# axruff/cuda-flow3d

Hardware: AMD Instinct MI355X
Metric: Mvoxels/s full pyramid solve (higher is better)
Workload: dtype f32; 1 GPU; 512^3 synthetic translated-Gaussian float32 pair (BASELINE config 4), full coarse-to-fine pyramid (40 levels x 40 outer x 5 inner, alpha 7.5, median 5^3, Gaussian sigma 2), frames resident in HBM (value = device-resident rate); parallelism=1 GPU

## Files before the change

### cuda-flow3d_amd/__init__.py

```python
import atexit
import collections
import contextlib
import ctypes as C
import os
import weakref

import numpy as np

_HERE = os.path.dirname(os.path.abspath(__file__))
_LIBDIR = os.environ.get("F3D_LIBDIR") or os.path.join(_HERE, "lib")

DEFAULT_PARAMS = dict(
    warp_levels_count=40, warp_scale_factor=0.95, outer_iterations_count=40, inner_iterations_count=5,
    equation_alpha=7.5, equation_smoothness=0.001, equation_data=0.001, median_radius=5, gaussian_sigma=2.0,
)


class F3dError(RuntimeError):
    pass


class Size4(C.Structure):
    _fields_ = [("width", C.c_size_t), ("height", C.c_size_t), ("depth", C.c_size_t), ("pitch", C.c_size_t)]

# ... 291 lines not shown
        "f3d_flow_create": [C.POINTER(C.c_void_p)], "f3d_flow_initialize": [C.c_void_p, _sz, _sz, _sz],
        "f3d_flow_compute": [C.c_void_p, _fp, _fp, pp, C.c_int, _fp, _fp, _fp],
        "f3d_flow_upload": [C.c_void_p, _fp, _fp],
        "f3d_flow_compute_resident": [C.c_void_p, pp, C.c_int, _fp],
        "f3d_flow_download": [C.c_void_p, _fp, _fp, _fp],
        "f3d_flow_container": [C.c_void_p, C.POINTER(Size4)], "f3d_flow_destroy": [C.c_void_p],
        "f3d_flow_set_level_stats": [C.c_void_p, C.c_int], "f3d_flow_level_stat_count": [C.c_void_p, C.POINTER(_sz)],
        "f3d_flow_level_stat": [C.c_void_p, _sz, C.POINTER(LevelStat)],
        "f3d_flow_final_residual": [C.c_void_p, C.POINTER(C.c_double), C.POINTER(C.c_double)],
        "f3d_flow_trajectory_begin": [C.c_void_p], "f3d_flow_trajectory_append": [C.c_void_p],
        "f3d_flow_trajectory_download": [C.c_void_p, _fp, _fp, _fp, C.POINTER(C.c_ulonglong)],
        "f3d_flow_trajectory_end": [C.c_void_p],
        "f3d_flow_strain_compute": [C.c_void_p, C.c_int, C.c_uint, C.POINTER(_fp), C.POINTER(StrainStats)],
        "f3d_flow_strain_end": [C.c_void_p],
        "f3d_flow_window_strain_compute": [C.c_void_p, C.c_int, C.c_uint, C.c_uint, C.c_uint, C.POINTER(_fp),
                                           C.POINTER(WindowStrainStats)],
        "f3d_flow_window_strain_end": [C.c_void_p],
        "f3d_flow_principal_compute": [C.c_void_p, C.c_int, C.c_uint, C.POINTER(_fp), C.POINTER(PrincipalStats)],
        "f3d_flow_principal_end": [C.c_void_p],
        "f3d_flow_polar_compute": [C.c_void_p, C.c_int, C.c_uint, C.POINTER(_fp), C.POINTER(PolarStats)],
        "f3d_flow_polar_end": [C.c_void_p],
        "f3d_flow_window_principal_compute": [C.c_void_p, C.c_int, C.c_uint, C.c_uint, C.c_uint, C.POINTER(_fp),
                                              C.POINTER(PrincipalStats)],
        "f3d_flow_window_principal_end": [C.c_void_p],
        "f3d_flow_window_polar_compute": [C.c_void_p, C.c_int, C.c_uint, C.c_uint, C.c_uint, C.POINTER(_fp), C.POINTER(PolarStats)],
        "f3d_flow_window_polar_end": [C.c_void_p],
        "f3d_flow_inverse_compute": [C.c_void_p, C.c_int, C.c_uint, C.c_float, C.POINTER(_fp), C.POINTER(InverseStats)],
        "f3d_flow_inverse_end": [C.c_void_p],
        "f3d_flow_match_compute": [C.c_void_p, C.c_int, C.c_uint, C.c_uint, C.c_float, C.POINTER(_fp), C.POINTER(CorrelationStats)],
        "f3d_flow_match_end": [C.c_void_p],
        "f3d_motion_solve": [C.POINTER(MotionSums), C.c_int, C.POINTER(MotionFit)],
        "f3d_motion_solve_labels": [C.POINTER(MotionSums), _sz, C.c_int, C.c_ulonglong, C.POINTER(C.c_double), C.POINTER(MotionFit),
                                    C.POINTER(C.c_int)],
        "f3d_flow_motion_compute": [C.c_void_p, C.c_int, C.c_int, C.c_float, C.POINTER(_fp), C.POINTER(MotionFit),
                                    C.POINTER(MotionResidual)],
        "f3d_flow_motion_end": [C.c_void_p],
        "f3d_flow_label_motion_compute": [C.c_void_p, C.c_int, C.POINTER(C.c_int), _sz, C.c_int, C.c_ulonglong, C.POINTER(_fp),
                                          C.POINTER(MotionFit), C.POINTER(C.c_int), C.POINTER(C.c_double), C.POINTER(LabelInfo)],
        "f3d_flow_label_motion_end": [C.c_void_p],
        "f3d_contact_kinematics": [C.POINTER(Contact), _sz, C.POINTER(_sz), C.POINTER(MotionFit), C.POINTER(C.c_int), _sz, C.c_ulonglong,
                                   C.POINTER(ContactKinematics)],
        "f3d_flow_contacts_compute": [C.c_void_p, C.c_int, C.POINTER(C.c_int), _sz, C.POINTER(C.POINTER(Contact)), C.POINTER(_sz),
                                      C.POINTER(ContactInfo)],
        "f3d_flow_contacts_end": [C.c_void_p],
        "f3d_flow_labels_compute": [C.c_void_p, _dp, C.c_float, C.c_float, C.c_ulonglong, C.POINTER(C.POINTER(C.c_ulonglong)), C.POINTER(_sz),
                                    C.POINTER(ComponentInfo)],
        "f3d_flow_labels_split": [C.c_void_p, _dp, C.c_float, C.c_float, C.c_ulonglong, C.c_ulonglong, C.POINTER(C.POINTER(C.c_ulonglong)),
                                  C.POINTER(_sz), C.POINTER(SplitInfo)],
        "f3d_flow_labels_end": [C.c_void_p], "f3d_flow_labels_download": [C.c_void_p, C.POINTER(C.c_int)],
        "f3d_flow_validate_compute": [C.c_void_p, C.c_int, C.c_uint, C.c_float, C.c_float, C.c_uint, C.c_uint, C.c_uint, C.c_float,
                                      C.POINTER(_fp), C.POINTER(ValidateStats)],
        "f3d_flow_validate_end": [C.c_void_p],
        "f3d_op_create": [C.POINTER(C.c_void_p), C.c_char_p], "f3d_op_initialize": [C.c_void_p, C.POINTER(Size4)],
        "f3d_op_execute": [C.c_void_p, C.POINTER(C.c_char_p), C.POINTER(C.c_void_p), _sz],
        "f3d_op_execute_batch": [C.c_void_p, C.POINTER(C.c_char_p), C.POINTER(C.c_void_p), C.POINTER(_sz), _sz],
        "f3d_op_set_slab": [C.c_void_p, _slabp], "f3d_op_destroy": [C.c_void_p],
        "f3d_level_geometry": [_sz, _sz, _sz, C.c_float, C.c_int, C.POINTER(Size4), _fp, _fp, _fp],
        "f3d_gaussian_taps": [C.c_float, _fp, _sz, C.POINTER(_sz)],
        "f3d_raw_read_u8": [C.c_char_p, _sz, _sz, _sz, _fp], "f3d_raw_read_f32": [C.c_char_p, _sz, _sz, _sz, _fp],
        "f3d_raw_write_u8": [C.c_char_p, _fp, _sz, _sz, _sz], "f3d_raw_write_f32": [C.c_char_p, _fp, _sz, _sz, _sz],
        "f3d_vtk_write_flow": [C.c_char_p, _fp, _fp, _fp, _sz, _sz, _sz],
        "f3d_synth_pair": [_sz, _sz, _sz, _fp, _fp],
        "f3d_synth_planes": [_sz, _sz, _sz, _sz, _sz, _fp, _fp, _fp],
        "f3d_slabflow_create": [C.POINTER(C.c_void_p), C.c_int, C.POINTER(C.c_int), C.c_int, C.c_int],
        "f3d_slabflow_initialize": [C.c_void_p, _sz, _sz, _sz],
        "f3d_slabflow_compute": [C.c_void_p, _fp, _fp, pp, _fp, _fp, _fp],
        "f3d_slabflow_upload": [C.c_void_p, _fp, _fp],
        "f3d_slabflow_compute_resident": [C.c_void_p, pp, _fp],
        "f3d_slabflow_download": [C.c_void_p, _fp, _fp, _fp],
        "f3d_slabflow_overlapped_iterations": [C.c_void_p, C.POINTER(_sz)],
        "f3d_slabflow_batched_exchanges": [C.c_void_p, C.POINTER(_sz)],
        "f3d_slabflow_gathered_warps": [C.c_void_p, C.POINTER(_sz)],
        "f3d_slabflow_stage_exchanges": [C.c_void_p, C.POINTER(_sz)],
        "f3d_slabflow_set_exchange_per_stage": [C.c_void_p, C.c_int],
        "f3d_slabflow_destroy": [C.c_void_p],
        "f3d_plan_owned": [C.c_int, C.c_int, C.c_int, C.POINTER(C.c_int), C.POINTER(C.c_int)],
        "f3d_plan_exchange": [C.c_int] * 5 + [C.POINTER(C.c_int)] * 5 + [C.c_int],
        "f3d_plan_resample_source": [C.c_int] * 4 + [C.POINTER(C.c_int)] * 2,
        "f3d_volume_wrap": [C.POINTER(C.c_void_p), _fp, _sz, _sz, _sz], "f3d_volume_destroy": [C.c_void_p],
        "f3d_op_solve_p_last": [C.c_void_p, C.POINTER(C.c_int), C.POINTER(C.c_int), C.POINTER(C.c_int), C.POINTER(_sz), C.POINTER(C.c_int)],
        "f3d_op_solve_p_fused_weights": [C.c_void_p, C.POINTER(C.c_int)],
        "f3d_plan_solve_piecemeal": [_sz, _sz, _sz, C.c_int, C.c_int, C.c_int, C.c_int, C.c_int] + [C.POINTER(C.c_int)] * 5,
        "f3d_plan_sweeps": [C.c_int] * 4 + [C.POINTER(C.c_int)] * 2 + [C.c_int],
        "f3d_pair8_plan": [C.c_int] * 7 + [C.POINTER(C.c_longlong)],
        "f3d_pair8_decode": [C.c_int] * 4 + [C.POINTER(C.c_longlong)] + [C.c_int] * 5 + [C.POINTER(C.c_int)] * 2,
        "f3d_pair8_plan_wide": [C.c_int] * 7 + [C.POINTER(C.c_longlong)],
        "f3d_pair8_decode_wide": [C.c_int] * 4 + [C.POINTER(C.c_longlong)] + [C.c_int] * 5 + [C.POINTER(C.c_int)] * 2,
        "f3d_pflow_create": [C.POINTER(C.c_void_p)], "f3d_pflow_initialize": [C.c_void_p, _sz, _sz, _sz],
        "f3d_pflow_compute": [C.c_void_p, _fp, _fp, _sz, _sz, _sz, pp, C.c_int, _fp, _fp, _fp, _fp],
        "f3d_pflow_stats": [C.c_void_p, C.POINTER(_sz), C.POINTER(_sz), C.POINTER(_sz)], "f3d_pflow_destroy": [C.c_void_p],
        "f3d_pflow_set_resident": [C.c_void_p, C.c_int], "f3d_pflow_set_full_pipeline": [C.c_void_p, C.c_int], "f3d_pflow_originals_on_device": [C.c_void_p, C.POINTER(C.c_int)],
        "f3d_pflow_operator_seconds": [C.c_void_p, C.POINTER(C.c_double)],
        "f3d_pflow_levels_registered_inside": [C.c_void_p, C.POINTER(_sz)],
        "f3d_pflow_levels_with_constants_on_device": [C.c_void_p, C.POINTER(_sz)],
        "f3d_host_shutdown": [],
    }
    for name, args in sig.items():
        try:
            fn = getattr(L, name)
        except AttributeError:
            if os.environ.get("F3D_LIBDIR"):
                continue
            raise
        fn.argtypes = args
        fn.restype = C.c_int
    L.f3d_flow_default_params.argtypes = [pp]
    L.f3d_flow_default_params.restype = None
    L.f3d_op_name.argtypes = [C.c_void_p]
    L.f3d_op_name.restype = C.c_char_p
    L.f3d_max_warp_level.argtypes = [_sz, _sz, _sz, C.c_float]
    L.f3d_max_warp_level.restype = _sz
    L.f3d_volume_object.argtypes = [C.c_void_p]
    L.f3d_volume_object.restype = C.c_void_p
    L.f3d_volume_data.argtypes = [C.c_void_p]
    L.f3d_volume_data.restype = C.c_void_p
    L.f3d_piecemeal_budget_bytes.argtypes = []
    L.f3d_piecemeal_budget_bytes.restype = _sz
    if hasattr(L, "f3d_host_last_error"):
        L.f3d_host_last_error.argtypes = []
        L.f3d_host_last_error.restype = C.c_char_p
    _host = L
    return L


def shutdown():
    HostVolume.release_all()
    if _host is not None:
        _host.f3d_host_shutdown()
    elif _hip is not None and _hip.f3d_is_initialized():
        _hip.f3d_comm_destroy()
        _hip.f3d_shutdown()


atexit.register(shutdown)


def check(status, what="f3d call"):
    if status != 0:
        msg = hip().f3d_last_error()
        raise F3dError(f"{what} failed: {msg.decode() if msg else 'status %d' % status}")


def _host_check(status, what):
    if status != 0:
        msg = host().f3d_host_last_error()
        raise F3dError(f"{what} failed: {msg.decode() if msg else 'status %d' % status}")


def _entry(name, argtypes, what):
    try:
        fn = getattr(hip(), name)
    except AttributeError:
        raise F3dError(f"{os.path.join(_LIBDIR, 'libf3d_hip.so')} has no {name}: this device library cannot {what}") from None
    fn.argtypes = argtypes
    fn.restype = C.c_int
    return fn


def solve_sweep_add_entry():
    return _entry("f3d_solve_sweep_add", [_dp] * 10 + [_sz] * 3 + [C.c_float] * 4 + [_dp] * 3 + [_slabp],
                  "add the increments to the flow inside the last sweep")


def _compose_entry():
    return _entry("f3d_compose_flow", [_dp] * 6 + [_sz] * 3 + [C.POINTER(C.c_ulonglong)], "compose flows into a trajectory")


def _strain_entry():
    return _entry("f3d_flow_strain", [_dp] * 3 + [_dpp, C.c_uint] + [_sz] * 3 + [C.POINTER(StrainStats)], "compute strain fields")


def _window_strain_entry():
    return _entry("f3d_window_strain", [_dp] * 3 + [_dpp, C.c_uint, C.c_uint, C.c_uint] + [_sz] * 3 + [C.POINTER(WindowStrainStats)],
                  "compute strain fields over a window")


def _principal_entry():
    return _entry("f3d_principal_strain", [_dp] * 3 + [_dpp, C.c_uint] + [_sz] * 3 + [C.POINTER(PrincipalStats)],
                  "compute principal strains")


def _polar_entry():
    return _entry("f3d_polar_decomposition", [_dp] * 3 + [_dpp, C.c_uint] + [_sz] * 3 + [C.POINTER(PolarStats)],
                  "compute local rotations and stretches")


def _principal_from_gradient_entry():
    return _entry("f3d_principal_from_gradient", [_dpp, _dpp, C.c_uint] + [_sz] * 3 + [C.POINTER(PrincipalStats)],
                  "compute principal strains of a stored gradient")


def _polar_from_gradient_entry():
    return _entry("f3d_polar_from_gradient", [_dpp, _dpp, C.c_uint] + [_sz] * 3 + [C.POINTER(PolarStats)],
                  "compute local rotations and stretches of a stored gradient")


def _inverse_entry():
    return _entry("f3d_invert_displacement", [_dp] * 7 + [_sz] * 3 + [C.c_uint, C.c_float, C.POINTER(InverseStats)],
                  "invert displacements")


def _carry_entry():
    return _entry("f3d_carry_field", [_dp] * 5 + [_sz] * 3 + [C.c_uint, C.POINTER(C.c_ulonglong)],
                  "carry fields through a displacement")


def _correlation_entry():
    return _entry("f3d_local_correlation", [_dp] * 2 + [_dpp, C.c_uint, C.c_uint, C.c_float] + [_sz] * 3 + [C.POINTER(CorrelationStats)],
                  "compute the local correlation of two volumes")


def _motion_entry():
    what = "fit or remove the motion of a displacement"
    return (_entry("f3d_motion_sums", [_dp] * 4 + [C.c_float] + [_sz] * 3 + [C.POINTER(MotionSums)], what),
            _entry("f3d_remove_motion", [_dp] * 6 + [C.POINTER(MotionFit)] + [_sz] * 3 + [C.POINTER(MotionResidual)], what))


_LABEL_MOTION_WHAT = "fit or remove the motion of the labels of a segmentation"


def _label_sums_entry():
    return _entry("f3d_label_motion_sums", [_dp] * 4 + [_sz, _dp, C.c_float] + [_sz] * 3 + [C.POINTER(MotionSums), C.POINTER(LabelInfo)],
                  _LABEL_MOTION_WHAT)


def _label_remove_entry():
    return _entry("f3d_remove_label_motion", [_dp] * 4 + [_sz, C.POINTER(MotionFit), C.POINTER(C.c_int)] + [_dp] * 3 + [_sz] * 3 +
                  [C.POINTER(MotionResidual)], _LABEL_MOTION_WHAT)


def _label_motion_entry():
    return _label_sums_entry(), _label_remove_entry()


def _contacts_entry():
    return _entry("f3d_label_contacts", [_dp] * 4 + [_sz] * 5 + [C.POINTER(Contact), C.POINTER(ContactInfo)],
                  "find the contacts between the labels of a segmentation")


def _components_entry():
    return _entry("f3d_label_components", [_dp, C.c_float, C.c_float, C.c_ulonglong, _dp] + [_sz] * 3 +
                  [C.POINTER(C.c_ulonglong), _sz, C.POINTER(ComponentInfo)], "label the connected bodies of a thresholded volume")


def _nearest_entry():
    return _entry("f3d_nearest_seed", [_dp, C.c_uint, C.c_uint] + [_dp] * 3 + [_sz] * 3 + [C.POINTER(NearestInfo)],
# ... 821 lines not shown
    _fields_ = [("min", C.c_float), ("max", C.c_float), ("avg", C.c_float)]


class HostVolume:
    _storage = {}

    def __init__(self, array, pin=False):
        a = np.ascontiguousarray(array, dtype=np.float32)
        if a.ndim != 3:
            raise ValueError("volume must be [z, y, x]")
        if pin and a.nbytes < (32 << 20):
            import mmap
            own = np.frombuffer(mmap.mmap(-1, max(a.nbytes, mmap.PAGESIZE)), dtype=np.float32, count=a.size).reshape(a.shape)
            own[...] = a
            a = own
        if a.ctypes.data in HostVolume._storage:
            raise ValueError("this array is already wrapped by another HostVolume")
        self._h = C.c_void_p()
        d, h, w = a.shape
        check(host().f3d_volume_wrap(C.byref(self._h), a.ctypes.data_as(_fp), w, h, d), "f3d_volume_wrap")
        entry = [a, False]
        HostVolume._storage[a.ctypes.data] = entry
        if pin:
            try:
                check(hip().f3d_init(-1), "f3d_init")
                check(hip().f3d_host_register(C.c_void_p(a.ctypes.data), a.nbytes), "f3d_host_register")
            except Exception:
                self.destroy()
                raise
            entry[1] = True
        self._finalizer = weakref.finalize(self, HostVolume._release, self._h.value)

    @staticmethod
    def _release(handle):
        if not handle or _host is None:
            return
        cur = _host.f3d_volume_data(C.c_void_p(handle))
        _host.f3d_volume_destroy(C.c_void_p(handle))
        entry = HostVolume._storage.pop(cur, None)
        if entry is not None and entry[1] and _hip is not None and _hip.f3d_is_initialized():
            _hip.f3d_host_unregister(C.c_void_p(cur))

    @classmethod
    def release_all(cls):
        for addr, entry in list(cls._storage.items()):
            if entry[1] and _hip is not None and _hip.f3d_is_initialized():
                _hip.f3d_host_unregister(C.c_void_p(addr))
            entry[1] = False

    @property
    def object(self):
        return host().f3d_volume_object(self._h)

    @property
    def array(self):
        return HostVolume._storage[host().f3d_volume_data(self._h)][0]

    def destroy(self):
        if self._h:
            fin = getattr(self, "_finalizer", None)
            if fin is not None:
                fin.detach()
            HostVolume._release(self._h.value)
            self._h = C.c_void_p()


def plan_solve_piecemeal(budget_bytes, width, height, depth, inner_iterations, outer_iterations, forced_outer_per_pass=0,
                         overlap_mode=0):
    out = [C.c_int() for _ in range(5)]
    check(host().f3d_plan_solve_piecemeal(budget_bytes, width, height, depth, inner_iterations, outer_iterations,
                                          forced_outer_per_pass, overlap_mode, *[C.byref(o) for o in out]))
    return tuple(o.value for o in out)


def plan_sweeps(inner, fused, tri, carry):
    cap = max(1, inner)
    sweeps, weights = (C.c_int * cap)(), (C.c_int * cap)()
    n = host().f3d_plan_sweeps(inner, int(bool(fused)), int(bool(tri)), int(bool(carry)), sweeps, weights, cap)
    if n < 0:
        raise F3dError("f3d_plan_sweeps failed")
    return [(sweeps[i], bool(weights[i])) for i in range(n)]


Pair8Plan = collections.namedtuple("Pair8Plan", "A a b zc_a zc_b wgs cost tiles")


def pair8_plan(width, rows, planes, ty, zc_limit=None, per_round=0, fold=False):
    out = (C.c_longlong * 8)()
    check(host().f3d_pair8_plan(width, rows, planes, ty, planes if zc_limit is None else zc_limit, per_round, int(bool(fold)), out))
    return Pair8Plan(*[int(v) for v in out])


def pair8_decode(width, rows, ty, fold, plan, xcd_remap, z_lo, z_hi):
    cut = (C.c_longlong * 8)(*plan)
    grid = C.c_int()
    args = (width, rows, ty, int(bool(fold)), cut, int(bool(xcd_remap)), z_lo, z_hi)
    check(host().f3d_pair8_decode(*args, 0, 0, None, C.byref(grid)))
    out = np.empty((grid.value, 6), np.int32)
    check(host().f3d_pair8_decode(*args, 0, grid.value, out.ctypes.data_as(C.POINTER(C.c_int)), None))
    return out


Pair8WidePlan = collections.namedtuple("Pair8WidePlan", "classes cost wgs tiles")


def pair8_plan_wide(width, rows, planes, ty, zc_limit=None, per_round=0, fold=False):
    out = (C.c_longlong * 12)()
    check(host().f3d_pair8_plan_wide(width, rows, planes, ty, planes if zc_limit is None else zc_limit, per_round, int(bool(fold)), out))
    v = [int(x) for x in out]
    return Pair8WidePlan(tuple(tuple(v[i:i + 3]) for i in (0, 3, 6) if v[i]), v[10], v[9], v[11])


def pair8_decode_wide(width, rows, ty, fold, plan, xcd_remap, z_lo, z_hi):
    classes = [c for c in plan.classes] + [(0, 0, 0)] * (3 - len(plan.classes))
    cut = (C.c_longlong * 9)(*[x for c in classes for x in c])
    grid = C.c_int()
    args = (width, rows, ty, int(bool(fold)), cut, int(bool(xcd_remap)), z_lo, z_hi)
    check(host().f3d_pair8_decode_wide(*args, 0, 0, None, C.byref(grid)))
    out = np.empty((grid.value, 6), np.int32)
    check(host().f3d_pair8_decode_wide(*args, 0, grid.value, out.ctypes.data_as(C.POINTER(C.c_int)), None))
    return out


class Operation:

    def __init__(self, name):
        self._h = C.c_void_p()
        if host().f3d_op_create(C.byref(self._h), name.encode()) != 0:
            raise F3dError(f"unknown operation {name!r}")
        self.values = {}

    @property
    def name(self):
        return host().f3d_op_name(self._h).decode()

    def initialize(self, containers=None):
        if containers is None:
            return host().f3d_op_initialize(self._h, None) == 0
        s = containers.size4
        return host().f3d_op_initialize(self._h, C.byref(s)) == 0

    def set_slab(self, slab):
        self._slab = slab
        host().f3d_op_set_slab(self._h, C.byref(slab) if slab is not None else None)

    def execute(self, **params):
        store = {}
        volumes = {}
        for k, v in params.items():
            if isinstance(v, HostVolume):
                volumes[k] = v
            elif k in _PTR_KEYS:
                store[k] = _dp(v)
            elif k in _SIZE_T_KEYS:
                store[k] = _sz(v)
            elif k in _FLOAT_KEYS:
                store[k] = C.c_float(v)
            elif k in _SIZE4_KEYS:
                store[k] = Size4(v[0], v[1], v[2], 0) if not isinstance(v, Size4) else v
            elif k == "max_mag":
                store[k] = _sz(v)
            elif k == "stat":
                store[k] = v
            elif k == "flow_update":
                store[k] = C.c_bool(bool(v))
            else:
# ... 546 lines not shown
```

### cuda-flow3d_amd/csrc/f3d_solve.hip

```cpp
#include <cmath>
#include <cstdio>
#include <algorithm>
#include <cstdlib>
#include <type_traits>

#include "f3d_internal.h"
#include "f3d_pair8_plan.h"

namespace {

constexpr int kLanes = 64;
static_assert(kLanes == kPair8Lanes, "f3d_pair8_plan.h counts tile columns of one wave");

__device__ __forceinline__ float lane_left(float v)
{
  const int i = __builtin_bit_cast(int, v);
  return __builtin_bit_cast(float, __builtin_amdgcn_update_dpp(i, i, 0x138 , 0xf, 0xf, false));
}
__device__ __forceinline__ float lane_right(float v)
{
  const int i = __builtin_bit_cast(int, v);
  return __builtin_bit_cast(float, __builtin_amdgcn_update_dpp(i, i, 0x130 , 0xf, 0xf, false));
}

// ... 1404 lines not shown
}

namespace {
int pair8_fd(const char* who, bool with_weights, const f3d_devptr (&in)[12], size_t width, size_t height, size_t depth, float hx, float hy,
             float hz, float alpha, float eps_s, float eps_d, const f3d_devptr (&out)[5], const f3d_slab* slab, int keep_below = 0,
             int keep_above = 0)
{
  F3dGeo g;
  if (!f3d::make_geo(&g, width, height, depth, slab, who)) return 1;
  if (g.W < 2 || g.H < 2 || g.D < 2) return f3d::fail("%s: every dimension must be at least 2", who);
  if (!pair_weights_finite(hx, hy, hz, alpha)) return f3d::fail("%s: alpha / h^2 must be finite and not negative (alpha %g, h %g %g %g)", who, alpha, hx, hy, hz);
  if (g.pitch % kLanes != 0) return f3d::fail("%s: the container pitch must be a multiple of 256 bytes (f3d_alloc_pitched gives that)", who);
  if (with_weights && (out[3] == in[8] || out[4] == in[9] || out[3] == in[9] || out[4] == in[8]))
    return f3d::fail("%s: phi_next / ksi_next must not alias phi / ksi (other tiles still read them)", who);
  if (g.z_lo == g.z_hi) return 0;
  if (!slab_reach_ok(g, 2, who)) return 1;
  PairArgs a = {};
  a.keep_below = with_weights && keep_below != 0;
  a.keep_above = with_weights && keep_above != 0;
  static const int plain_division = std::getenv("F3D_UDIV") && std::atoi(std::getenv("F3D_UDIV")) == 0;
  a.plain_division = plain_division;
  for (int i = 0; i < 12; ++i) a.in[i] = f3d_ptr<const float>(in[i]);
  for (int i = 0; i < 5; ++i) a.out[i] = f3d_ptr<float>(out[i]);
  a.hx = hx; a.hy = hy; a.hz = hz;
  a.alpha = alpha;
  a.eps_s = eps_s;
  a.eps_d = eps_d;
  const int kid = with_weights ? F3D_K_SWEEP_PHI_KSI : F3D_K_SWEEP2;
  f3d::prof_begin(kid, static_cast<size_t>(g.W) * g.H * (g.z_hi - g.z_lo));
  const int rows = pair8_rows(g);
  if (with_weights) {
    if (rows == 12) launch_pair8<PAIR_SP, 12, true>(a, g, tuning().zchunk, tuning().xcd_remap);
    else if (rows == 4) launch_pair8<PAIR_SP, 4, true>(a, g, tuning().zchunk, tuning().xcd_remap);
    else launch_pair8<PAIR_SP, 8, true>(a, g, tuning().zchunk, tuning().xcd_remap);
  } else {
    if (rows == 12) launch_pair8<PAIR_SS, 12, true>(a, g, tuning().zchunk, tuning().xcd_remap);
    else if (rows == 4) launch_pair8<PAIR_SS, 4, true>(a, g, tuning().zchunk, tuning().xcd_remap);
    else launch_pair8<PAIR_SS, 8, true>(a, g, tuning().zchunk, tuning().xcd_remap);
  }
  f3d::prof_end(kid);
  F3D_HIP(hipGetLastError());
  return 0;
}
}

int f3d_solve_sweep2_fd(f3d_devptr fx, f3d_devptr fy, f3d_devptr fz, f3d_devptr ft, f3d_devptr flow_u, f3d_devptr flow_v, f3d_devptr flow_w,
                        f3d_devptr flow_du, f3d_devptr flow_dv, f3d_devptr flow_dw, f3d_devptr phi, f3d_devptr ksi, size_t width,
                        size_t height, size_t depth, float hx, float hy, float hz, float equation_alpha, f3d_devptr temp_du,
                        f3d_devptr temp_dv, f3d_devptr temp_dw, const f3d_slab* slab)
{
  F3D_REQUIRE_READY("f3d_solve_sweep2_fd");
  const f3d_devptr in[12] = {fx, fy, flow_u, flow_v, flow_w, flow_du, flow_dv, flow_dw, phi, ksi, fz, ft};
  const f3d_devptr out[5] = {temp_du, temp_dv, temp_dw, 0, 0};
  return pair8_fd("f3d_solve_sweep2_fd", false, in, width, height, depth, hx, hy, hz, equation_alpha, 0.f, 0.f, out, slab);
}

int f3d_solve_sweep_phi_ksi_fd(f3d_devptr fx, f3d_devptr fy, f3d_devptr fz, f3d_devptr ft, f3d_devptr flow_u, f3d_devptr flow_v,
                               f3d_devptr flow_w, f3d_devptr flow_du, f3d_devptr flow_dv, f3d_devptr flow_dw, f3d_devptr phi,
                               f3d_devptr ksi, size_t width, size_t height, size_t depth, float hx, float hy, float hz,
                               float equation_alpha, float equation_smoothness, float equation_data, f3d_devptr temp_du,
                               f3d_devptr temp_dv, f3d_devptr temp_dw, f3d_devptr phi_next, f3d_devptr ksi_next, const f3d_slab* slab)
{
  F3D_REQUIRE_READY("f3d_solve_sweep_phi_ksi_fd");
  const f3d_devptr in[12] = {fx, fy, flow_u, flow_v, flow_w, flow_du, flow_dv, flow_dw, phi, ksi, fz, ft};
  const f3d_devptr out[5] = {temp_du, temp_dv, temp_dw, phi_next, ksi_next};
  return pair8_fd("f3d_solve_sweep_phi_ksi_fd", true, in, width, height, depth, hx, hy, hz, equation_alpha, equation_smoothness,
                  equation_data, out, slab);
}

int f3d_solve_sweep_phi_ksi_edges_fd(f3d_devptr fx, f3d_devptr fy, f3d_devptr fz, f3d_devptr ft, f3d_devptr flow_u, f3d_devptr flow_v,
                                     f3d_devptr flow_w, f3d_devptr flow_du, f3d_devptr flow_dv, f3d_devptr flow_dw, f3d_devptr phi,
                                     f3d_devptr ksi, size_t width, size_t height, size_t depth, float hx, float hy, float hz,
                                     float equation_alpha, float equation_smoothness, float equation_data, f3d_devptr temp_du,
                                     f3d_devptr temp_dv, f3d_devptr temp_dw, f3d_devptr phi_next, f3d_devptr ksi_next, const f3d_slab* slab,
                                     int keep_below, int keep_above)
{
  F3D_REQUIRE_READY("f3d_solve_sweep_phi_ksi_edges_fd");
  const f3d_devptr in[12] = {fx, fy, flow_u, flow_v, flow_w, flow_du, flow_dv, flow_dw, phi, ksi, fz, ft};
  const f3d_devptr out[5] = {temp_du, temp_dv, temp_dw, phi_next, ksi_next};
  return pair8_fd("f3d_solve_sweep_phi_ksi_edges_fd", true, in, width, height, depth, hx, hy, hz, equation_alpha, equation_smoothness,
                  equation_data, out, slab, keep_below, keep_above);
}

int f3d_fused_launches_march_along_y(size_t width, size_t height, size_t depth)
{
  F3dGeo g = {};
  const f3d_size4& c = f3d::container();
  g.W = static_cast<int>(width); g.H = static_cast<int>(height); g.D = static_cast<int>(depth);
  g.Hc = static_cast<int>(c.height); g.pitch = static_cast<int>(c.pitch / sizeof(float));
  g.z_base = 0; g.z_lo = 0; g.z_hi = g.D;
  if (g.pitch <= 0 || g.pitch % kLanes != 0 || !pair8_enabled()) return 0;
  return pair8_ymarch_rows(g) != 0 ? 1 : 0;
}

int f3d_solve_sweep3(f3d_devptr frame_0, f3d_devptr frame_1, f3d_devptr flow_u, f3d_devptr flow_v, f3d_devptr flow_w,
                     f3d_devptr flow_du, f3d_devptr flow_dv, f3d_devptr flow_dw, f3d_devptr phi, f3d_devptr ksi, size_t width,
                     size_t height, size_t depth, float hx, float hy, float hz, float equation_alpha, f3d_devptr temp_du,
                     f3d_devptr temp_dv, f3d_devptr temp_dw, const f3d_slab* slab)
{
  F3D_REQUIRE_READY("f3d_solve_sweep3");
  const f3d_devptr in[10] = {frame_0, frame_1, flow_u, flow_v, flow_w, flow_du, flow_dv, flow_dw, phi, ksi};
  const f3d_devptr out[5] = {temp_du, temp_dv, temp_dw, 0, 0};
  return tri_launch("f3d_solve_sweep3", false, in, width, height, depth, hx, hy, hz, equation_alpha, 0.f, 0.f, out, slab);
}

int f3d_solve_sweep2_phi_ksi(f3d_devptr frame_0, f3d_devptr frame_1, f3d_devptr flow_u, f3d_devptr flow_v, f3d_devptr flow_w,
                             f3d_devptr flow_du, f3d_devptr flow_dv, f3d_devptr flow_dw, f3d_devptr phi, f3d_devptr ksi, size_t width,
                             size_t height, size_t depth, float hx, float hy, float hz, float equation_alpha, float equation_smoothness,
                             float equation_data, f3d_devptr temp_du, f3d_devptr temp_dv, f3d_devptr temp_dw, f3d_devptr phi_next,
                             f3d_devptr ksi_next, const f3d_slab* slab)
{
  F3D_REQUIRE_READY("f3d_solve_sweep2_phi_ksi");
  const f3d_devptr in[10] = {frame_0, frame_1, flow_u, flow_v, flow_w, flow_du, flow_dv, flow_dw, phi, ksi};
  const f3d_devptr out[5] = {temp_du, temp_dv, temp_dw, phi_next, ksi_next};
  return tri_launch("f3d_solve_sweep2_phi_ksi", true, in, width, height, depth, hx, hy, hz, equation_alpha, equation_smoothness,
                    equation_data, out, slab);
}

}
```

### cuda-flow3d_amd/csrc/f3d_solve_pair8.h

```cpp

enum { PAIR_SS = 0, PAIR_SP = 1 };

struct PairArgs {
  const float* in[12];
  float* out[5];
  float hx, hy, hz, alpha;
  float eps_s, eps_d;
  int plain_division;
  int keep_below, keep_above;
  double r4[3], r2[3];
  float d4[3], d2[3];
  float w[3];
  float eps_s2, eps_d2;
  int fdivs_ok, sdivs_ok;
};

inline bool pair_weights_finite(float hx, float hy, float hz, float alpha)
{
  for (float h : {hx, hy, hz}) {
    const float w = alpha / (h * h);
    if (!(w - w == 0.f) || std::signbit(w)) return false;
  }
  return true;
}
inline bool host_divisor_ok(float d) { return d >= 0x1p-20f && d <= 0x1p20f; }
inline void pair_consts(PairArgs& a)
{
  const float h[3] = {a.hx, a.hy, a.hz};
  a.fdivs_ok = a.sdivs_ok = 1;
  for (int i = 0; i < 3; ++i) {
    a.d4[i] = 4.f * h[i];
    a.d2[i] = 2.f * h[i];
    a.r4[i] = 1.0 / static_cast<double>(a.d4[i]);
    a.r2[i] = 1.0 / static_cast<double>(a.d2[i]);
    a.w[i] = a.alpha / (h[i] * h[i]);
    a.fdivs_ok = a.fdivs_ok && host_divisor_ok(a.d4[i]);
    a.sdivs_ok = a.sdivs_ok && host_divisor_ok(a.d4[i]) && host_divisor_ok(a.d2[i]);
  }
  a.eps_s2 = a.eps_s * a.eps_s;
  a.eps_d2 = a.eps_d * a.eps_d;
  if (a.plain_division) a.fdivs_ok = a.sdivs_ok = 0;
}

template <int TY, int NA = 10, bool FD = false, bool TIGHT = false>
struct Pair8Lds {
  static constexpr int NR = TY + (TIGHT ? 0 : 2);
  static constexpr int NJ = TY + (TIGHT ? 0 : 4);
  static constexpr int NK = (NJ + 3) / 4;
  static constexpr int NJP = NJ;
  static constexpr int NS = FD ? 7 : NA;
  static constexpr int kHaloLanes = NS * 2 * NJ;
  static constexpr int NH = (kHaloLanes + 63) / 64;
  static constexpr int kRowFloats = NS * NJP * 64;
  static constexpr int kHaloOff = kRowFloats;
  static constexpr int kSlotFloats = kRowFloats + NH * 256;
  static constexpr int kSlots = 3;
  static constexpr int kPerPlane = NS * NK + NH;
  static_assert(kPerPlane <= 63, "s_waitcnt vmcnt(kPerPlane): the counter has six bits");
  static constexpr int NC = FD ? 5 : 0;
  static constexpr int NRC = TY + 2;
  static constexpr int NKC = (NRC + 3) / 4;
  static constexpr int kCHaloLanes = NC * 2 * TY;
  static constexpr int NHC = (kCHaloLanes + 63) / 64;
  static constexpr int kCRowFloats = NC * NRC * 64;
  static constexpr int kCHaloOff = kCRowFloats;
  static constexpr int kCSlotFloats = FD ? kCRowFloats + NHC * 256 : 4;
  static constexpr int kCSlots = 2;
  static constexpr int kPerPlaneC = NC * NKC + NHC;
};

template <typename T>
__device__ __forceinline__ T* uniform_ptr(T* p)
{
  const unsigned long long v = reinterpret_cast<unsigned long long>(p);
  const unsigned lo = __builtin_amdgcn_readfirstlane(static_cast<unsigned>(v));
  const unsigned hi = __builtin_amdgcn_readfirstlane(static_cast<unsigned>(v >> 32));
  return reinterpret_cast<T*>((static_cast<unsigned long long>(hi) << 32) | lo);
}

__device__ __forceinline__ float opaque(float seed)
{
  asm volatile("" : "+v"(seed));
  return seed;
}

__device__ __forceinline__ int fresh_lane()
{
  int l;
  asm volatile("v_mbcnt_lo_u32_b32 %0, -1, 0\n\tv_mbcnt_hi_u32_b32 %0, -1, %0" : "=v"(l));
  return l;
}

__device__ __forceinline__ void dma16(const float* base, unsigned byte_off, float* lds_dst)
{
  const unsigned m0v = static_cast<unsigned>(reinterpret_cast<unsigned long>((LdsFloat*)lds_dst));
  asm volatile("s_nop 4\n\tglobal_load_lds_dwordx4 %0, %1" ::"v"(byte_off), "s"(base), "{m0}"(m0v) : "memory");
}
__device__ __forceinline__ void dma16_lane(const float* lane_addr, float* lds_dst)
{
  const unsigned m0v = static_cast<unsigned>(reinterpret_cast<unsigned long>((LdsFloat*)lds_dst));
  asm volatile("s_nop 0\n\tglobal_load_lds_dwordx4 %0, off" ::"v"(lane_addr), "{m0}"(m0v) : "memory");
}

struct CarryP {
  float fx, fy, fz, ft;
  float D[9];
};

constexpr unsigned kWeightLo = 0x0d800000u, kWeightHi = 0x71800000u;
__device__ __forceinline__ float weight_fast(float a, float& s_out)
{
  const float y = __builtin_amdgcn_rsqf(a);
  const float h = 0.5f * y;
  const float s0 = a * y;
  const float s = __builtin_fmaf(__builtin_fmaf(-s0, s0, a), h, s0);
  s_out = s;
  const float t = s + s;
  return __builtin_fmaf(__builtin_fmaf(-t, h, 1.f), h, h);
}
__device__ __forceinline__ bool weight_fast_ok(float a, float s)
{
  return (__float_as_uint(a) - kWeightLo) <= (kWeightHi - kWeightLo) && (__float_as_uint(s) & 0x7fffffu) != 0x7fffffu;
}
__device__ __forceinline__ float weight_ieee(float a) { return 1.f / (2.f * sqrtf(a)); }

__device__ __forceinline__ void phi_ksi_stage2(const CarryP& k, const S3& xm, const S3& xp, const S3& ym, const S3& yp,
                                               const S3& zm, const S3& zp, float du, float dv_c, float dw,
                                               const SolveDivs& dv, float eps_s2, float eps_d2, float& phi, float& ksi,
                                               bool counts = true, bool fast_weights = true)
{
  float q[9] = {k.D[0] + xp.u - xm.u, k.D[1] + yp.u - ym.u, k.D[2] + zp.u - zm.u,
                k.D[3] + xp.v - xm.v, k.D[4] + yp.v - ym.v, k.D[5] + zp.v - zm.v,
                k.D[6] + xp.w - xm.w, k.D[7] + yp.w - ym.w, k.D[8] + zp.w - zm.w};
  if (__builtin_expect(dv.ok && udiv_all_safe(q), 1)) {
#pragma unroll
    for (int c = 0; c < 3; ++c) {
      q[3 * c + 0] = udiv(q[3 * c + 0], dv.x2);
      q[3 * c + 1] = udiv(q[3 * c + 1], dv.y2);
      q[3 * c + 2] = udiv(q[3 * c + 2], dv.z2);
    }
  } else {
#pragma unroll
    for (int c = 0; c < 3; ++c) {
      q[3 * c + 0] = q[3 * c + 0] / dv.x2.d;
      q[3 * c + 1] = q[3 * c + 1] / dv.y2.d;
      q[3 * c + 2] = q[3 * c + 2] / dv.z2.d;
    }
  }
  const float dux = q[0], duy = q[1], duz = q[2], dvx = q[3], dvy = q[4], dvz = q[5], dwx = q[6], dwy = q[7], dwz = q[8];
  const float a_phi = dux * dux + duy * duy + duz * duz + dvx * dvx + dvy * dvy + dvz * dvz + dwx * dwx + dwy * dwy + dwz * dwz + eps_s2;
  const float fx = k.fx, fy = k.fy, fz = k.fz, ft = k.ft;
  const float J11 = fx * fx, J22 = fy * fy, J33 = fz * fz;
  const float J12 = fx * fy, J13 = fx * fz, J23 = fy * fz;
  const float J14 = fx * ft, J24 = fy * ft, J34 = fz * ft, J44 = ft * ft;
  float s = (J11 * du + J12 * dv_c + J13 * dw + J14) * du + (J12 * du + J22 * dv_c + J23 * dw + J24) * dv_c +
            (J13 * du + J23 * dv_c + J33 * dw + J34) * dw + (J14 * du + J24 * dv_c + J34 * dw + J44);
  s = static_cast<float>(s > 0) * s;
  const float a_ksi = s + eps_d2;
  float s_phi, s_ksi;
  const float w_phi = weight_fast(a_phi, s_phi), w_ksi = weight_fast(a_ksi, s_ksi);
  const bool lane_ok = !counts || (weight_fast_ok(a_phi, s_phi) && weight_fast_ok(a_ksi, s_ksi));
  if (__builtin_expect(fast_weights && __builtin_amdgcn_ballot_w64(!lane_ok) == 0, 1)) {
    phi = w_phi;
    ksi = w_ksi;
  } else {
    phi = weight_ieee(a_phi);
    ksi = weight_ieee(a_ksi);
  }
}


template <int MODE, int TY, int ABL, bool FD, bool YM, bool TIGHT, bool FOLDS = false>
__device__ __forceinline__ void pair8_body(const PairArgs& a, const F3dGeo& g, const Pair8Cut& cut, int ntx, int nty, int xcd_remap)
{
  static_assert(!FOLDS || (!YM && !TIGHT && ABL == 0), "two row bands per tile: z-marching product builds only");
  static_assert(!(YM && FD), "the frame-derivative launchers march along z only");
  static_assert(!TIGHT || (YM && ABL == 0), "a tile without halo rows holds every row of the volume: thin volumes marched along y");
  constexpr int RH = TIGHT ? 0 : 1;
  const int RDIM = YM ? g.D : g.H;
  const int MDIM = YM ? g.H : g.D;
  const int m_lo = YM ? 0 : g.z_lo, m_hi = YM ? g.H : g.z_hi;
  constexpr int NA = FD ? 12 : 10;
  using L = Pair8Lds<TY, NA, FD, TIGHT>;
  constexpr int NR = L::NR, NJ = L::NJ, NK = L::NK, NJP = L::NJP, NH = L::NH;
  static_assert(TY <= 32, "the column wave holds one halo voxel per lane: 2 x TY <= 64");
  __shared__ __attribute__((aligned(16))) float ring[L::kSlots][L::kSlotFloats];
  __shared__ __attribute__((aligned(16))) float cring[L::kCSlots][L::kCSlotFloats];
  constexpr int SB = FD ? 2 : 0;
  __shared__ float img1[2][3][NR][kLanes];
  __shared__ float hc1[2][3][2][32];
  __shared__ float img3[(ABL & 64) ? 3 : 1][(ABL & 64) ? NR : 1][(ABL & 64) ? kLanes : 1];

  Pair8Wg wg;
  if (!pair8_decode(static_cast<int>(blockIdx.x), cut, ntx, nty, FOLDS, xcd_remap, m_lo, m_hi, (ABL & 64) ? 1 : 0, wg)) return;
  const int tx = wg.tx, ty = wg.ty;
  const bool folded = wg.folded;

  auto tile_body = [&](auto fold_c) __attribute__((always_inline)) {
  constexpr bool FOLD = decltype(fold_c)::value;
  int lane = threadIdx.x;
  const int r = __builtin_amdgcn_readfirstlane(static_cast<int>(threadIdx.y));
  const bool colw = r == NR;
  const bool loader = r == NR + 1;
  const int z0 = wg.z0, z1 = wg.z1;
  const int qs = z0 > 0 ? z0 - 1 : 0;
  const int qe = z1 < MDIM ? z1 : MDIM - 1;
  const int q_end = z1 < MDIM ? qe : qe + 1;
  const int p_last = qe + 1;
  const int x0 = tx * kLanes;
  const int y0 = ty * TY;
  const bool left_face = tx == 0;
  const bool right_face = x0 + kLanes >= g.W;
  const bool tile_at_x_face = __builtin_amdgcn_readfirstlane(static_cast<int>(left_face || right_face)) != 0;
  const bool col_at_x_face = __builtin_amdgcn_readfirstlane(static_cast<int>(left_face || right_face || x0 + kLanes == g.W - 1)) != 0;

  const int st_lo = (a.keep_below && z0 == m_lo) ? z0 - 1 : z0;
  const int st_hi = (a.keep_above && z1 == m_hi) ? z1 + 1 : z1;
  const int zb = qs > 0 ? qs - 1 : 0;
  const unsigned z_stride_b = static_cast<unsigned>(g.Hc) * static_cast<unsigned>(g.pitch) * 4u;
  const unsigned y_stride_b = static_cast<unsigned>(g.pitch) * 4u;
  const unsigned plane_b = YM ? y_stride_b : z_stride_b;
  const unsigned row_b = YM ? z_stride_b : y_stride_b;
  const size_t base_off = YM ? static_cast<size_t>(zb) * static_cast<size_t>(g.pitch) : f3d_row(g, 0, zb);

  if (loader) {
    __builtin_amdgcn_s_setprio(3);
    const float* base[NA];
#pragma unroll
    for (int i = 0; i < NA; ++i) base[i] = uniform_ptr(a.in[i] + base_off);
    const bool bandb = FOLD && (lane & 15) >= 8;
    const int seg = bandb ? (lane & 15) - 8 : (lane & 15);
    unsigned rowb[NK];
    bool rowv[NK];
#pragma unroll
    for (int k = 0; k < NK; ++k) {
      const int j = 4 * k + (lane >> 4);
      rowv[k] = j < NJ;
      const int yrow = f3d_clampi(f3d_mir(y0 + (bandb ? TY : 0) - 2 * RH + (rowv[k] ? j : 0), RDIM), 0, RDIM - 1);
      rowb[k] = static_cast<unsigned>(yrow) * row_b + static_cast<unsigned>(x0 + 4 * seg) * 4u;
    }
    const float* hptr[NH];
    bool hv[NH];
#pragma unroll
    for (int h = 0; h < NH; ++h) {
      const int lp = 64 * h + lane;
      hv[h] = lp < L::kHaloLanes;
      const int lq = hv[h] ? lp : 0;
      const int arr = lq / (2 * NJ) + SB;
      const int s = (lq / NJ) & 1;
      const int j = lq % NJ;
      const float* b = base[SB];
#pragma unroll
      for (int i = SB + 1; i < SB + L::NS; ++i)
        if (arr == i) b = base[i];
      const int yrow = f3d_clampi(f3d_mir(y0 + (FOLD && s ? TY : 0) - 2 * RH + j, RDIM), 0, RDIM - 1);
      const int xc = FOLD ? x0 - 4 : s == 0 ? (left_face ? 0 : x0 - 4) : (right_face ? x0 + kLanes - 4 : x0 + kLanes);
      hptr[h] = b + static_cast<size_t>(yrow) * static_cast<size_t>(row_b >> 2) + xc;
    }
    auto issue = [&](int p) {
      float* slot = &ring[(p - qs + 1) % L::kSlots][0];
      const int zz = f3d_mir(p, MDIM);
      const unsigned poff = static_cast<unsigned>(__builtin_amdgcn_readfirstlane(static_cast<int>(static_cast<unsigned>(zz - zb) * plane_b)));
      unsigned off[NK];
#pragma unroll
      for (int k = 0; k < NK; ++k) off[k] = rowb[k] + poff;
#pragma unroll
      for (int i = 0; i < L::NS; ++i) {
#pragma unroll
        for (int k = 0; k < NK; ++k) {
          if (NJ % 4 == 0 || rowv[k]) dma16(base[SB + i], off[k], slot + (i * NJP + 4 * k) * kLanes);
        }
      }
#pragma unroll
      for (int h = 0; h < NH; ++h)
        if (hv[h]) dma16_lane(hptr[h] + (poff >> 2), slot + L::kHaloOff + h * 256);
    };
    constexpr int NKC = FD ? L::NKC : 1, NHC = FD ? L::NHC : 1;
    constexpr int kCIn[5] = {0, 1, 9, 10, 11};
    unsigned crowb[NKC];
    bool crowv[NKC];
    const float* chptr[NHC];
    bool chv[NHC];
    if constexpr (FD) {
#pragma unroll
      for (int k = 0; k < NKC; ++k) {
        const int j = 4 * k + (lane >> 4);
        crowv[k] = j < L::NRC;
        const int yrow = f3d_clampi(f3d_mir(y0 + (bandb ? TY : 0) - 1 + (crowv[k] ? j : 0), RDIM), 0, RDIM - 1);
        crowb[k] = static_cast<unsigned>(yrow) * row_b + static_cast<unsigned>(x0 + 4 * seg) * 4u;
      }
#pragma unroll
      for (int h = 0; h < NHC; ++h) {
        const int lp = 64 * h + lane;
        chv[h] = lp < L::kCHaloLanes;
        const int lq = chv[h] ? lp : 0;
        const int arr = lq / (2 * TY);
        const int s = (lq / TY) & 1;
        const int j = lq % TY;
        const float* b = base[kCIn[0]];
#pragma unroll
        for (int i = 1; i < 5; ++i)
          if (arr == i) b = base[kCIn[i]];
        const int yrow = f3d_clampi(f3d_mir(y0 + (FOLD && s ? TY : 0) + j, RDIM), 0, RDIM - 1);
        const int xc = FOLD ? x0 - 4 : s == 0 ? (left_face ? 0 : x0 - 4) : (right_face ? x0 + kLanes - 4 : x0 + kLanes);
        chptr[h] = b + static_cast<size_t>(yrow) * static_cast<size_t>(row_b >> 2) + xc;
      }
    }
    auto issue_c = [&](int p) {
      if constexpr (FD) {
        float* slot = &cring[(p - qs) & 1][0];
        const int zz = f3d_mir(p, MDIM);
        const unsigned poff = static_cast<unsigned>(__builtin_amdgcn_readfirstlane(static_cast<int>(static_cast<unsigned>(zz - zb) * plane_b)));
#pragma unroll
        for (int i = 0; i < 5; ++i) {
#pragma unroll
          for (int k = 0; k < NKC; ++k)
            if (L::NRC % 4 == 0 || crowv[k]) dma16(base[kCIn[i]], crowb[k] + poff, slot + (i * L::NRC + 4 * k) * kLanes);
        }
#pragma unroll
        for (int h = 0; h < NHC; ++h)
          if (chv[h]) dma16_lane(chptr[h] + (poff >> 2), slot + L::kCHaloOff + h * 256);
      }
    };
    issue(qs - 1);
    if (!(ABL & 32)) {
      issue(qs);
      issue(qs + 1);
      issue_c(qs);
      issue_c(qs + 1);
    }
    asm volatile("s_waitcnt vmcnt(0)" ::: "memory");
    __syncthreads();
    if (ABL & 8) return;
    for (int q = qs; q <= q_end; ++q) {
      __syncthreads();
      if (!(ABL & 1)) {
        if (q == qs && q + 2 <= p_last) issue(q + 2);
        if (q + 3 <= p_last) {
          issue_c(q + 2);
          issue(q + 3);
          asm volatile("s_waitcnt vmcnt(%0)" ::"n"(L::kPerPlane) : "memory");
          continue;
        }
        if (q + 2 <= p_last) issue_c(q + 2);
      }
      asm volatile("s_waitcnt vmcnt(0)" ::: "memory");
    }
    return;
  }

  FDivs fdivs;
  fdivs.x4 = UDiv{a.r4[0], a.d4[0]}; fdivs.y4 = UDiv{a.r4[1], a.d4[1]}; fdivs.z4 = UDiv{a.r4[2], a.d4[2]};
  fdivs.ok = a.fdivs_ok != 0;
  SolveDivs sdivs = {};
  if (MODE == PAIR_SP) {
    sdivs.x2 = UDiv{a.r2[0], a.d2[0]}; sdivs.y2 = UDiv{a.r2[1], a.d2[1]}; sdivs.z2 = UDiv{a.r2[2], a.d2[2]};
    sdivs.x4 = fdivs.x4; sdivs.y4 = fdivs.y4; sdivs.z4 = fdivs.z4;
    sdivs.ok = a.sdivs_ok != 0;
  }

  const int y = y0 - RH + r;
  const int yy = f3d_clampi(f3d_mir(y, RDIM), 0, RDIM - 1);
  const int side = lane < 32 ? 0 : 1;
  const int x = FOLD ? x0 + (lane & 31) : x0 + lane;
  const bool core = r >= RH && r < RH + TY;
  const bool owner = core && x < g.W && (FOLD && side ? y + TY : y) < RDIM;
  const int jr = r + RH;
  const int jr_m = (TIGHT && y == 0) ? jr + 1 : jr - 1;
  const int jr_p = (TIGHT && y == RDIM - 1) ? jr - 1 : jr + 1;
  const int r_ym = y == 0 ? r + 1 : r - 1;
  const int r_yp = y == RDIM - 1 ? r - 1 : r + 1;
  const int r_ymb = r - 1;
  const int r_ypb = y + TY == RDIM - 1 ? r - 1 : r + 1;
  const unsigned xb = static_cast<unsigned>(x) * 4u + (FOLD && side ? static_cast<unsigned>(TY) * row_b : 0u);
  const bool cactive = (lane & 31) < TY;
  const int crow = cactive ? (lane & 31) : TY - 1;
  const int cy = y0 + crow + (FOLD && side ? TY : 0);
  const int cx = FOLD || side == 0 ? x0 - 1 : x0 + kLanes;
  const int jc = crow + 2 * RH;
  const int jc_m = (TIGHT && cy == 0) ? jc + 1 : jc - 1;
  const int jc_p = (TIGHT && cy == RDIM - 1) ? jc - 1 : jc + 1;
  const int e_near = FOLD || side == 0 ? 3 : 0;
  const int e_far = FOLD || side == 0 ? 2 : 1;
  auto left_or = [&](float v, float edge) __attribute__((always_inline)) {
    const float s = lane_left_or(v, edge);
    if constexpr (FOLD) return lane == 32 ? edge : s;
    else return s;
  };

  float* obase[5];
#pragma unroll
  for (int i = 0; i < 5; ++i) obase[i] = (i < 3 || MODE == PAIR_SP) ? uniform_ptr(a.out[i] + base_off) : nullptr;
  auto rowoff = [&](int yrow, int zz) __attribute__((always_inline)) {
    return static_cast<unsigned>(__builtin_amdgcn_readfirstlane(
        static_cast<int>(static_cast<unsigned>(zz - zb) * plane_b + static_cast<unsigned>(yrow) * row_b)));
  };

  float seedv = static_cast<float>(lane) * 0.01f + 1.f;
  auto fake_raw = [&](PlaneRegs& p) __attribute__((always_inline)) {
    p.f0 = opaque(seedv); p.f1 = opaque(seedv); p.u = opaque(seedv); p.v = opaque(seedv); p.w = opaque(seedv);
    p.su = opaque(seedv); p.dv = opaque(seedv); p.dw = opaque(seedv); p.phi = opaque(seedv); p.ksi = opaque(seedv);
    p.fz = opaque(seedv); p.ft = opaque(seedv);
  };
  auto row_raw = [&](PlaneRegs& p, const float* slot, int j, bool with_ksi, const float* cs = nullptr) __attribute__((always_inline)) {
    if (ABL & 8) return fake_raw(p);
    const float* d = slot + j * kLanes + lane;
    constexpr int st = NJP * kLanes;
    if (!FD) {
      p.f0 = d[F0 * st];
      p.f1 = d[F1 * st];
    }
    p.u = d[(U - SB) * st]; p.v = d[(V - SB) * st]; p.w = d[(Wf - SB) * st];
    p.su = d[(DU - SB) * st]; p.dv = d[(DV - SB) * st]; p.dw = d[(DW - SB) * st]; p.phi = d[(PHI - SB) * st];
    if (!FD && with_ksi) p.ksi = d[9 * st];
    if (FD && !with_ksi) p.f0 = p.f1 = 0.f;
    if (FD && with_ksi) {
      const float* c = cs + (j - 1) * kLanes + lane;
      constexpr int ct = L::NRC * kLanes;
      p.f0 = c[0 * ct]; p.f1 = c[1 * ct]; p.ksi = c[2 * ct]; p.fz = c[3 * ct]; p.ft = c[4 * ct];
    }
  };
  auto halo_raw = [&](PlaneRegs& p, const float* slot, int s, int j, int e, bool with_ksi, const float* cs = nullptr) __attribute__((always_inline)) {
    if (ABL & 8) return fake_raw(p);
    const float* d = slot + L::kHaloOff + (s * NJ + j) * 4 + e;
    constexpr int st = 2 * NJ * 4;
    if (!FD) {
      p.f0 = d[F0 * st];
      p.f1 = d[F1 * st];
    }
    p.u = d[(U - SB) * st]; p.v = d[(V - SB) * st]; p.w = d[(Wf - SB) * st];
    p.su = d[(DU - SB) * st]; p.dv = d[(DV - SB) * st]; p.dw = d[(DW - SB) * st]; p.phi = d[(PHI - SB) * st];
    if (!FD && with_ksi) p.ksi = d[9 * st];
    if (FD && !with_ksi) p.f0 = p.f1 = 0.f;
    if (FD && with_ksi) {
      const float* c = cs + L::kCHaloOff + (s * TY + (j - 2)) * 4 + e;
      constexpr int ct = 2 * TY * 4;
      p.f0 = c[0 * ct]; p.f1 = c[1 * ct]; p.ksi = c[2 * ct]; p.fz = c[3 * ct]; p.ft = c[4 * ct];
    }
  };

  S3 hM = {0.f, 0.f, 0.f}, hC = {0.f, 0.f, 0.f};
  float hC_dv = 0.f, hC_dw = 0.f;
  Carry kC = {};
  Carry kC2 = {};
  CarryP pC = {};

  Face6 nYm = {}, nYp = {}, nX = {};
  S3 nDy = {0.f, 0.f, 0.f}, nXr = {0.f, 0.f, 0.f};
  Face6 nIn = {};
  S3 nInr = {0.f, 0.f, 0.f};
  auto fetch_neighbours = [&](auto colw_c, const float* S) __attribute__((always_inline)) {
    constexpr bool CW = decltype(colw_c)::value;
    PlaneRegs T0, T1, T2;
    if constexpr (CW) {
      PlaneRegs T;
      const float* d = S + jc * kLanes + (side ? (FOLD ? 32 : kLanes - 1) : 0);
      constexpr int st = NJP * kLanes;
      if (ABL & 8) {
        fake_raw(T);
      } else {
        if (!FD) {
          T.f0 = d[F0 * st];
          T.f1 = d[F1 * st];
        } else {
          T.f0 = T.f1 = 0.f;
        }
        T.u = d[(U - SB) * st]; T.v = d[(V - SB) * st]; T.w = d[(Wf - SB) * st];
        T.su = d[(DU - SB) * st]; T.dv = d[(DV - SB) * st]; T.dw = d[(DW - SB) * st]; T.phi = d[(PHI - SB) * st];
      }
      nInr = {T.u, T.v, T.w};
      plane_finish(T);
      nIn = plane_face(T);
    }
    if constexpr (CW) {
      halo_raw(T0, S, side, jc_m, e_near, false);
// ... 30 lines not shown

    float r_du = 0.f, r_dv = 0.f, r_dw = 0.f;
    Carry kN;
    CarryP pN;
    {
      Face6 xm, xp;
      const Face6 ym = nYm, yp = nYp;
      S3 rxm = {}, rxp = {};
      int vx, vy;
      if constexpr (CW) {
        halo_raw(P, Sp, side, jc, e_near, true, Cp);
        plane_finish(P);
        const S3 router = nXr;
        const Face6 outer = nX;
        const S3 rinner = nInr;
        const Face6 inner = nIn;
#pragma unroll
        for (int i = 0; i < kNL; ++i) {
          xm.v[i] = !FOLD && side ? inner.v[i] : outer.v[i];
          xp.v[i] = !FOLD && side ? outer.v[i] : inner.v[i];
        }
        rxm = !FOLD && side ? rinner : router;
        rxp = !FOLD && side ? router : rinner;
        vx = cx;
        vy = cy;
        if (cx == g.W - 1) {
          xp = xm;
          rxp = rxm;
        }
      } else {
        row_raw(P, Sp, jr, true, Cp);
        plane_finish(P);
        const S3 rx = nXr;
        const Face6 xf = nX;
        const Face6 cf = plane_face(C);
#pragma unroll
        for (int i = 0; i < kNL; ++i) {
          xm.v[i] = left_or(cf.v[i], xf.v[i]);
          xp.v[i] = lane_right_or(cf.v[i], xf.v[i]);
        }
        if (MODE == PAIR_SP) {
          rxm = {left_or(C.u, rx.u), left_or(C.v, rx.v), left_or(C.w, rx.w)};
          rxp = {lane_right_or(C.u, rx.u), lane_right_or(C.v, rx.v), lane_right_or(C.w, rx.w)};
        }
        vx = x;
        vy = band ? y + TY : y;
        if (tile_at_x_face) {
          if (x == 0) {
            xm = xp;
            rxm = rxp;
          }
          if (x == g.W - 1) {
            xp = xm;
            rxp = rxm;
          }
        }
      }
      const Face6 cfc = plane_face(C);
      if (ABL & 2) {
        kN = Carry{};
        r_du = xm.v[0] + xp.v[1] + ym.v[2] + yp.v[3] + M.su + P.sv + C.ksi + rxm.u + nDy.v;
        r_dv = xm.v[4] + xp.v[5] + ym.v[0] + yp.v[1] + M.f0 + P.f1 + C.u + rxp.w + nDy.u;
        r_dw = xm.v[2] + xp.v[3] + ym.v[4] + yp.v[5] + M.phi + P.phi + C.dv + C.dw + C.v + C.w;
        kN.J12 = r_du; kN.d1 = r_dv; kN.pw[0] = r_dw;
      } else
      {
        const Face6 fM = plane_face(M), fP = plane_face(P);
        const bool row_p = vy < RDIM - 1, row_m = vy > 0, mar_p = q < MDIM - 1, mar_m = q > 0;
        constexpr bool FDA = FD || (ABL & 16) != 0;
        sweep_stage1<FDA, true>(xm, xp, YM ? fM : ym, YM ? fP : yp, YM ? ym : fM, YM ? yp : fP, cfc.v, C.u, C.v, C.w, C.dv, C.dw,
                                C.ksi, a.hx, a.hy, a.hz, fdivs, a.alpha, vx < g.W - 1, vx > 0, YM ? mar_p : row_p, YM ? mar_m : row_m,
                                YM ? row_p : mar_p, YM ? row_m : mar_m, r_du, r_dv, r_dw, kN, C.f0, C.f1, FD ? C.fz : C.phi,
                                FD ? C.ft : C.ksi, CW ? col_at_x_face : tile_at_x_face, a.w[0], a.w[1], a.w[2]);
      }
      pN.fx = kN.fx; pN.fy = kN.fy; pN.fz = kN.fz; pN.ft = kN.ft;
      {
        const S3 dRow = nDy, dMar = {P.u - M.u, P.v - M.v, P.w - M.w};
        const S3 dY = YM ? dMar : dRow, dZ = YM ? dRow : dMar;
        pN.D[0] = rxp.u - rxm.u; pN.D[1] = dY.u; pN.D[2] = dZ.u;
        pN.D[3] = rxp.v - rxm.v; pN.D[4] = dY.v; pN.D[5] = dZ.v;
        pN.D[6] = rxp.w - rxm.w; pN.D[7] = dY.w; pN.D[8] = dZ.w;
      }
    }
    const S3 sN = MODE == PAIR_SS ? S3{C.u + r_du, C.v + r_dv, C.w + r_dw} : S3{r_du, r_dv, r_dw};
    if (do1 && !(ABL & 8)) {
      if constexpr (CW) {
        if (cactive) {
          hc1[b][0][side][crow] = sN.u;
          hc1[b][1][side][crow] = sN.v;
          hc1[b][2][side][crow] = sN.w;
        }
      } else {
        img1[b][0][r][lane] = sN.u;
        img1[b][1][r][lane] = sN.v;
        img1[b][2][r][lane] = sN.w;
      }
    }
    if (MODE == PAIR_SP && do1 && owner && q >= st_lo && q < st_hi) {
      const unsigned off = xb + rowoff(yy, q);
      gst(obase[0], off, r_du);
      gst(obase[1], off, r_dv);
      gst(obase[2], off, r_dw);
    }

    const int t = q - 1;
    const bool do2 = !CW && core && t >= z0;
    float o0 = 0.f, o1 = 0.f, o2 = 0.f;
    if (do2) {
      const int pb = t & 1;
      S3 ym, yp, xm, xp, zm, zp;
      float eu, ev, ew;
      if (ABL & 8) {
        ym.u = opaque(seedv); ym.v = opaque(seedv); ym.w = opaque(seedv);
        yp.u = opaque(seedv); yp.v = opaque(seedv); yp.w = opaque(seedv);
        eu = opaque(seedv); ev = opaque(seedv); ew = opaque(seedv);
      } else {
        const int im = band ? r_ymb : r_ym, ip = band ? r_ypb : r_yp;
        ym.u = img1[pb][0][im][lane]; ym.v = img1[pb][1][im][lane]; ym.w = img1[pb][2][im][lane];
        yp.u = img1[pb][0][ip][lane]; yp.v = img1[pb][1][ip][lane]; yp.w = img1[pb][2][ip][lane];
        eu = hc1[pb][0][side][r - RH]; ev = hc1[pb][1][side][r - RH]; ew = hc1[pb][2][side][r - RH];
      }
      xm.u = left_or(hC.u, eu); xm.v = left_or(hC.v, ev); xm.w = left_or(hC.w, ew);
      xp.u = lane_right_or(hC.u, eu); xp.v = lane_right_or(hC.v, ev); xp.w = lane_right_or(hC.w, ew);
      zm = hM;
      zp = sN;
      if (tile_at_x_face) {
        if (x == 0) xm = xp;
        if (x == g.W - 1) xp = xm;
      }
      if (t == 0) zm = zp;
      if (t == MDIM - 1) zp = zm;
      if (ABL & 2) {
        o0 = xm.u + xp.v + ym.w + kC.J12;
        o1 = yp.u + zm.v + zp.w + kC.d1;
        o2 = xm.w + yp.v + zp.u + kC.pw[0] + hC_dv + hC_dw;
      } else if (MODE == PAIR_SS)
        sweep_stage2(kC, xm, xp, YM ? zm : ym, YM ? zp : yp, YM ? ym : zm, YM ? yp : zp, hC_dv, hC_dw, o0, o1, o2);
      else
        phi_ksi_stage2(pC, xm, xp, YM ? zm : ym, YM ? zp : yp, YM ? ym : zm, YM ? yp : zp, hC.u, hC.v, hC.w, sdivs, a.eps_s2,
                       a.eps_d2, o0, o1, owner, a.plain_division == 0);
    }
    if constexpr ((ABL & 64) != 0) {
      if (do2) {
        img3[0][r][lane] = o0; img3[1][r][lane] = o1; img3[2][r][lane] = o2;
        S3 ym, yp, xm, xp;
        ym.u = img3[0][r_ym][lane]; ym.v = img3[1][r_ym][lane]; ym.w = img3[2][r_ym][lane];
        yp.u = img3[0][r_yp][lane]; yp.v = img3[1][r_yp][lane]; yp.w = img3[2][r_yp][lane];
        const float eu = hc1[b][0][side][r - 1], ev = hc1[b][1][side][r - 1], ew = hc1[b][2][side][r - 1];
        xm.u = lane_left_or(o0, eu); xm.v = lane_left_or(o1, ev); xm.w = lane_left_or(o2, ew);
        xp.u = lane_right_or(o0, eu); xp.v = lane_right_or(o1, ev); xp.w = lane_right_or(o2, ew);
        const S3 zm = hM, zp = {o0, o1, o2};
        float p0, p1, p2;
        sweep_stage2(kC2, xm, xp, ym, yp, zm, zp, o1, o2, p0, p1, p2);
        o0 = p0; o1 = p1; o2 = p2;
      }
      kC2 = kC;
    }
    asm volatile("" ::"v"(o0), "v"(o1), "v"(o2), "v"(sN.u), "v"(sN.v), "v"(sN.w));
    hM = hC;
    hC = sN;
    hC_dv = r_dv;
    hC_dw = r_dw;
    kC = kN;
    pC = pN;
    if (do2 && owner) {
      const unsigned off = xb + rowoff(yy, t);
      if (MODE == PAIR_SS) {
        gst(obase[0], off, o0);
        gst(obase[1], off, o1);
        gst(obase[2], off, o2);
      } else {
        gst(obase[3], off, o0);
        gst(obase[4], off, o1);
      }
    }
    fetch_neighbours(colw_c, Sp);
  };

  __syncthreads();
  PlaneRegs A = {}, B = {}, Cc = {};
  const float* Sm = &ring[0][0];
  const float* S0 = &ring[1][0];
  using Slot0 = std::integral_constant<int, 0>;
  using Slot1 = std::integral_constant<int, 1>;
  using Slot2 = std::integral_constant<int, 2>;
  auto march = [&](auto colw_c) __attribute__((always_inline)) {
    constexpr bool CW = decltype(colw_c)::value;
    if constexpr (CW) {
      halo_raw(A, Sm, side, jc, e_near, false);
      halo_raw(B, S0, side, jc, e_near, true, &cring[0][0]);
    } else {
      row_raw(A, Sm, jr, false);
      row_raw(B, S0, jr, true, &cring[0][0]);
    }
    plane_finish(A);
    plane_finish(B);
    fetch_neighbours(colw_c, S0);
    int q = qs;
    for (; q + 2 <= q_end; q += 3) {
      step(colw_c, Slot2{}, A, B, Cc, q);
      step(colw_c, Slot0{}, B, Cc, A, q + 1);
      step(colw_c, Slot1{}, Cc, A, B, q + 2);
    }
    if (q <= q_end) step(colw_c, Slot2{}, A, B, Cc, q);
    if (q + 1 <= q_end) step(colw_c, Slot0{}, B, Cc, A, q + 1);
  };
  if (colw) march(std::true_type{});
  else march(std::false_type{});
  asm volatile("s_waitcnt vmcnt(0)" ::: "memory");
  };
  if constexpr (FOLDS) {
    if (__builtin_amdgcn_readfirstlane(static_cast<int>(folded))) return tile_body(std::true_type{});
  }
  tile_body(std::false_type{});
}

template <int MODE, int TY, int ABL = 0, bool FD = false, bool YM = false, bool FOLDS = false>
__global__ __launch_bounds__(kLanes*(TY + 4)) void k_pair8(PairArgs a, F3dGeo g, Pair8Cut cut, int ntx, int nty, int xcd_remap)
{
  pair8_body<MODE, TY, ABL, FD, YM, false, FOLDS>(a, g, cut, ntx, nty, xcd_remap);
}
template <int MODE, int TY>
__global__ __launch_bounds__(kLanes*(TY + 2)) __attribute__((amdgpu_waves_per_eu(4))) void k_pair8t(PairArgs a, F3dGeo g, Pair8Cut cut, int ntx,
                                                                                                   int nty, int xcd_remap)
{
  pair8_body<MODE, TY, 0, false, true, true>(a, g, cut, ntx, nty, xcd_remap);
}

inline Pair8Plan pair8_plan_launch_kept(int width, int rows, int planes, int ty, int zc_limit, long per_round, bool fold)
{
  struct Key {
    int width, rows, planes, ty, zc_limit, fold, plan;
    long per_round;
    bool operator==(const Key& o) const
    {
      return width == o.width && rows == o.rows && planes == o.planes && ty == o.ty && zc_limit == o.zc_limit && fold == o.fold &&
             plan == o.plan && per_round == o.per_round;
    }
  };
  thread_local Key keys[3] = {};
  thread_local Pair8Plan plans[3] = {};
  const char* pe = std::getenv("F3D_PAIR8_PLAN");
  const Key key = {width, rows, planes, ty, zc_limit, fold ? 1 : 0, pe ? pe[0] : 0, per_round};
  const int slot = ty <= 4 ? 0 : (ty <= 8 ? 1 : 2);
  if (!(keys[slot] == key)) {
    plans[slot] = pair8_plan_launch(width, rows, planes, ty, zc_limit, per_round, fold);
    keys[slot] = key;
  }
  return plans[slot];
}

inline Pair8Plan pair8_plan(const F3dGeo& g, int ty, long per_round = 256)
{
  return pair8_plan_launch_kept(g.W, g.H, g.z_hi - g.z_lo, ty, max_planes_per_chunk(g), pair8_per_round(per_round),
                                pair8_folds(g.W, g.H, ty));
}

inline int pair8_ymarch_rows(const F3dGeo& g)
{
  const char* e = std::getenv("F3D_PAIR8_YMARCH");
  const int mode = e ? std::atoi(e) : -1;
  if (mode == 0) return 0;
  if (g.z_base != 0 || g.z_lo != 0 || g.z_hi != g.D || g.D > 8 || g.D < 2 || g.H < 2) return 0;
  const unsigned long long bytes = static_cast<unsigned long long>(g.Hc) * static_cast<unsigned long long>(g.pitch) * 4ull *
                                   static_cast<unsigned long long>(g.D + 1);
  if (bytes >= 0xf0000000ull) return 0;
  const char* te = std::getenv("F3D_PAIR8_TIGHT");
  const bool tight = !(te && te[0] == '0');
  const int min_planes = tight ? 4 : 5;
  if (mode != 1 && (g.D < min_planes || g.H < 8 * g.D)) return 0;
  return g.D <= 4 ? 4 : (g.D == 5 ? 5 : 8);
}

template <int MODE, int TY, bool FD = false, bool YM = false, bool TIGHT = false>
void launch_pair8(const PairArgs& args, const F3dGeo& g, int force_zchunk, int xcd_remap)
{
  PairArgs a = args;
  pair_consts(a);
  const int rows = YM ? g.D : g.H;
  const int planes = YM ? g.H : g.z_hi - g.z_lo;
  const int ntx = (g.W + kLanes - 1) / kLanes;
  const int nty = (rows + TY - 1) / TY;
  const int zc_limit = YM ? planes : max_planes_per_chunk(g);
#ifdef F3D_LAB
  static const int abl = std::getenv("F3D_ABLATE8") ? std::atoi(std::getenv("F3D_ABLATE8")) : 0;
#else
  constexpr int abl = 0;
#endif
  const int fold = !YM && abl == 0 && pair8_folds(g.W, rows, TY) ? 1 : 0;
  const int tiles = pair8_tiles_per_chunk(ntx, nty, fold != 0);
  const long per_round = pair8_per_round(TIGHT ? 512 : 256);
  Pair8Cut cut = !YM && abl == 0 ? pair8_plan_launch_kept(g.W, rows, planes, TY, zc_limit, per_round, fold != 0).cut
                                 : pair8_plan_two(g.W, rows, planes, TY, zc_limit, per_round, fold != 0, false).cut;
  if (force_zchunk > 0) cut = pair8_uniform_cut(tiles, planes, std::min(force_zchunk, zc_limit));
  const dim3 grid(pair8_cut_grid(cut, xcd_remap), 1, 1), block(kLanes, TY + (TIGHT ? 2 : 4), 1);
  auto go = [&](auto kern) { hipLaunchKernelGGL(kern, grid, block, 0, f3d::stream(), a, g, cut, ntx, nty, xcd_remap); };
  if constexpr (!YM) {
    if (fold) return go(k_pair8<MODE, TY, 0, FD, false, true>);
  }
  if constexpr (YM && TIGHT) return go(k_pair8t<MODE, TY>);
  else if constexpr (YM) return go(k_pair8<MODE, TY, 0, false, true>);
  else if constexpr (FD) return go(k_pair8<MODE, TY, 0, true>);
  else {
#ifdef F3D_LAB
    if constexpr (TY == 12) {
      if (abl == 16) return go(k_pair8<MODE, TY, 16>);
    }
    if constexpr (MODE == PAIR_SS) {
      if (abl == 1) return go(k_pair8<MODE, TY, 1>);
      if (abl == 2) return go(k_pair8<MODE, TY, 2>);
      if (abl == 3) return go(k_pair8<MODE, TY, 3>);
      if (abl == 4) return go(k_pair8<MODE, TY, 4>);
      if (abl == 8) return go(k_pair8<MODE, TY, 8>);
      if (abl == 40) return go(k_pair8<MODE, TY, 40>);
      if constexpr (TY <= 8) {
        if (abl == 64) return go(k_pair8<MODE, TY, 64>);
      }
    }
#endif
    go(k_pair8<MODE, TY, 0>);
  }
}

template <int MODE>
bool launch_pair8_ymarch(const PairArgs& a, const F3dGeo& g, int force_zchunk, int xcd_remap)
{
  const char* e = std::getenv("F3D_PAIR8_TIGHT");
  const bool tight = !(e && e[0] == '0');
  switch (pair8_ymarch_rows(g)) {
    case 4:
      if (tight && g.D == 4) launch_pair8<MODE, 4, false, true, true>(a, g, force_zchunk, xcd_remap);
      else launch_pair8<MODE, 4, false, true>(a, g, force_zchunk, xcd_remap);
      return true;
    case 5:
      if (tight && g.D == 5) launch_pair8<MODE, 5, false, true, true>(a, g, force_zchunk, xcd_remap);
      else launch_pair8<MODE, 5, false, true>(a, g, force_zchunk, xcd_remap);
      return true;
    case 8: launch_pair8<MODE, 8, false, true>(a, g, force_zchunk, xcd_remap); return true;
    default: return false;
  }
}
```

### cuda-flow3d_amd/host/hip_utils.cpp

```cpp
#include "hip_utils.h"

#include <cstdlib>

bool InitDeviceContextWithFirstAvailableDevice()
{
  int count = 0;
  if (CheckDeviceError(f3d_device_count(&count))) return false;
  if (count == 0) {
    std::printf("There are no HIP capable devices.");
    return false;
  }
  if (CheckDeviceError(f3d_init(-1))) return false;
  char name[128];
  if (CheckDeviceError(f3d_device_name(name, sizeof(name)))) return false;
  std::printf("HIP Device: %s. Launch timeout: %s\n", name, "No");
  return true;
}

void CopyData3DtoDevice(Data3D& data3d, DevicePtr device_ptr, size_t device_height, size_t device_pitch)
{
  CheckDeviceError(f3d_copy3d_h2d(device_ptr, device_pitch, device_height, 0, data3d.DataPtr(), data3d.Width(),
                                  data3d.Height(), data3d.Depth()));
}

void CopyData3DFromDevice(DevicePtr device_ptr, Data3D& data3d, size_t device_height, size_t device_pitch)
{
  CheckDeviceError(f3d_copy3d_d2h(data3d.DataPtr(), data3d.Width(), data3d.Height(), data3d.Depth(), device_ptr,
                                  device_pitch, device_height, 0));
}

bool FusedSweepsEnabled()
{
  static const bool on = [] {
    const char* e = std::getenv("F3D_FUSED_SWEEPS");
    return !(e && e[0] == '0');
  }();
  return on;
}

bool FusedPhiKsiEnabled()
{
  static const bool on = [] {
    const char* e = std::getenv("F3D_FUSED_PHI_KSI");
    return !(e && e[0] == '0');
  }();
  return on;
}

bool FrameDerivativesEnabled()
{
  static const bool on = [] {
    const char* e = std::getenv("F3D_FRAME_DERIVATIVES");
    return !(e && e[0] == '0');
  }();
  return on;
}

bool ThreeStageLaunchesPay(size_t width, size_t height, size_t depth)
{
  static const bool on = [] {
    const char* e = std::getenv("F3D_TRI");
    return e && e[0] == '1';
  }();
  static const double max_voxels = [] {
    const char* e = std::getenv("F3D_TRI_MAX_VOXELS");
    return e ? std::atof(e) : 3.0e6;
  }();
  return on && static_cast<double>(width) * static_cast<double>(height) * static_cast<double>(depth) <= max_voxels;
}
```

### cuda-flow3d_amd/host/hip_utils.h

```cpp
#ifndef F3D_HOST_HIP_UTILS_H_
#define F3D_HOST_HIP_UTILS_H_

#include <cstdio>

#include "data_types.h"
#include "f3d.h"

#define CheckDeviceError(status) CheckDeviceErrorAt((status), __FILE__, __LINE__)
inline bool CheckDeviceErrorAt(int status, const char* file, int line)
{
  if (status != 0) {
    std::fprintf(stderr, "Device API error = %04d\n%s\n from file <%s>, line %i.\n", status, f3d_last_error(), file, line);
    return true;
  }
  return false;
}

class ProfilerRange {
 public:
  explicit ProfilerRange(const char* name) { f3d_range_push(name); }
  ~ProfilerRange() { f3d_range_pop(); }
  ProfilerRange(const ProfilerRange&) = delete;
  ProfilerRange& operator=(const ProfilerRange&) = delete;
};

bool InitDeviceContextWithFirstAvailableDevice();
void CopyData3DtoDevice(Data3D& data3d, DevicePtr device_ptr, size_t device_height, size_t device_pitch);
void CopyData3DFromDevice(DevicePtr device_ptr, Data3D& data3d, size_t device_height, size_t device_pitch);
bool FusedSweepsEnabled();
bool FusedPhiKsiEnabled();
bool FrameDerivativesEnabled();
bool ThreeStageLaunchesPay(size_t width, size_t height, size_t depth);

#endif
```

### cuda-flow3d_amd/host/host_capi.cpp

```cpp
#include <cstring>
#include <memory>
#include <new>
#include <string>
#include <vector>

#include "f3d_host.h"
#include "contact_kinematics.h"
#include "hip_utils.h"
#include "motion_fit.h"
#include "operations.h"
#include "operations_p.h"
#include "optical_flow.h"
#include "optical_flow_p.h"
#include "optical_flow_slab.h"
#include "synth.h"
#include "../csrc/f3d_pair8_plan.h"

struct f3d_flow_s {
  OpticalFlowE driver;
  bool device_ready = false;
  bool trajectory_started = false;
  bool zncc_of_held_flow = false;
  std::vector<f3d_contact> contacts;
  std::vector<unsigned long long> label_sizes;
// ... 658 lines not shown
{
  if (!flow) return 1;
  if (solve_passes) *solve_passes = flow->driver.LastSolvePasses();
  if (streamed_levels) *streamed_levels = flow->driver.LastStreamedLevels();
  if (resident_levels) *resident_levels = flow->driver.LastResidentLevels();
  return 0;
}

int f3d_pflow_levels_registered_inside(f3d_pflow flow, size_t* levels)
{
  if (!flow || !levels) return 1;
  *levels = flow->driver.LastLevelsRegisteredInside();
  return 0;
}

int f3d_pflow_levels_with_constants_on_device(f3d_pflow flow, size_t* levels)
{
  if (!flow || !levels) return 1;
  *levels = flow->driver.LastLevelsWithConstantsOnDevice();
  return 0;
}

int f3d_pflow_originals_on_device(f3d_pflow flow, int* yes)
{
  if (!flow || !yes) return 1;
  *yes = flow->driver.LastOriginalsOnDevice() ? 1 : 0;
  return 0;
}

int f3d_pflow_set_full_pipeline(f3d_pflow flow, int enabled)
{
  if (!flow) return 1;
  flow->driver.full_pipeline = enabled != 0;
  return 0;
}

int f3d_pflow_set_resident(f3d_pflow flow, int enabled)
{
  if (!flow) return 1;
  flow->driver.resident_coarse_levels = enabled != 0;
  return 0;
}

int f3d_pflow_operator_seconds(f3d_pflow flow, double* seconds6)
{
  if (!flow || !seconds6) return 1;
  for (int i = 0; i < 6; ++i) seconds6[i] = flow->driver.LastOperatorSeconds()[i];
  return 0;
}

int f3d_pflow_destroy(f3d_pflow flow)
{
  delete flow;
  return 0;
}

size_t f3d_piecemeal_budget_bytes(void) { return PiecemealBudgetBytes(); }

int f3d_plan_solve_piecemeal(size_t budget_bytes, size_t width, size_t height, int depth, int inner_iterations, int outer_iterations,
                             int forced_outer_per_pass, int overlap_mode, int* chunk, int* outer_per_pass, int* halo, int* max_planes,
                             int* overlapped)
{
  const SolvePiecemealPlan plan = PlanSolvePiecemeal(budget_bytes, width, height, depth, inner_iterations, outer_iterations,
                                                     forced_outer_per_pass, overlap_mode);
  if (overlapped) *overlapped = plan.overlapped ? 1 : 0;
  if (chunk) *chunk = plan.chunk;
  if (outer_per_pass) *outer_per_pass = plan.outer_per_pass;
  if (halo) *halo = plan.halo;
  if (max_planes) *max_planes = plan.max_planes;
  return 0;
}

int f3d_plan_sweeps(int inner, int fused, int tri, int carry, int* sweeps, int* next_weights, int capacity)
{
  const std::vector<SweepLaunch> cut = CutSweeps(inner, fused != 0, tri != 0, carry != 0);
  if (static_cast<int>(cut.size()) > capacity || (!cut.empty() && (!sweeps || !next_weights))) return -1;
  for (size_t i = 0; i < cut.size(); ++i) {
    sweeps[i] = cut[i].sweeps;
    next_weights[i] = cut[i].next_weights ? 1 : 0;
  }
  return static_cast<int>(cut.size());
}

int f3d_pair8_plan(int width, int rows, int planes, int ty, int zc_limit, int per_round, int fold, long long* plan)
{
  if (!plan || width < 1 || rows < 1 || planes < 1 || ty < 1 || zc_limit < 1) return 1;
  const Pair8Plan p = pair8_plan_dims(width, rows, planes, ty, zc_limit, per_round > 0 ? per_round : pair8_per_round(256), fold != 0);
  const long long v[8] = {p.cut.tiles_a, p.cut.chunks_a, p.cut.chunks_b, p.cut.zc_a, p.cut.zc_b, pair8_cut_wgs(p.cut), p.cost,
                          p.cut.tiles_a + p.cut.tiles_b};
  std::copy(v, v + 8, plan);
  return 0;
}

int f3d_pair8_decode(int width, int rows, int ty, int fold, const long long* plan, int xcd_remap, int z_lo, int z_hi, int first,
                     int count, int* out, int* grid)
{
  if (!plan || width < 1 || rows < 1 || ty < 1 || z_hi <= z_lo || first < 0 || count < 0 || (count && !out)) return 1;
  const int ntx = (width + kPair8Lanes - 1) / kPair8Lanes, nty = (rows + ty - 1) / ty;
  const int tiles = pair8_tiles_per_chunk(ntx, nty, fold != 0);
  const Pair8Cut cut = {static_cast<int>(plan[0]), static_cast<int>(plan[1]), static_cast<int>(plan[3]),
                        tiles - static_cast<int>(plan[0]), static_cast<int>(plan[2]), static_cast<int>(plan[4]), 0, 0, 0};
  if (cut.tiles_a < 0 || cut.tiles_b < 0 || (cut.tiles_a && (cut.chunks_a < 1 || cut.zc_a < 1)) ||
      (cut.tiles_b && (cut.chunks_b < 1 || cut.zc_b < 1)))
    return 1;
  if (grid) *grid = pair8_cut_grid(cut, xcd_remap);
  for (int i = 0; i < count; ++i) {
    Pair8Wg w;
    int* o = out + 6 * static_cast<size_t>(i);
    if (pair8_decode(first + i, cut, ntx, nty, fold != 0, xcd_remap, z_lo, z_hi, 0, w)) {
      o[0] = w.tile; o[1] = w.tx; o[2] = w.ty; o[3] = w.folded ? 1 : 0; o[4] = w.z0; o[5] = w.z1;
    } else {
      std::fill(o, o + 6, -1);
    }
  }
  return 0;
}

int f3d_pair8_plan_wide(int width, int rows, int planes, int ty, int zc_limit, int per_round, int fold, long long* plan)
{
  if (!plan || width < 1 || rows < 1 || planes < 1 || ty < 1 || zc_limit < 1) return 1;
  const Pair8Plan p = pair8_plan_launch(width, rows, planes, ty, zc_limit, per_round > 0 ? per_round : pair8_per_round(256), fold != 0);
  const Pair8Cut& c = p.cut;
  const long long v[12] = {c.tiles_a, c.chunks_a, c.zc_a, c.tiles_b, c.chunks_b, c.zc_b, c.tiles_c, c.chunks_c, c.zc_c,
                           pair8_cut_wgs(c), p.cost, c.tiles_a + c.tiles_b + c.tiles_c};
  std::copy(v, v + 12, plan);
  return 0;
}

int f3d_pair8_decode_wide(int width, int rows, int ty, int fold, const long long* plan, int xcd_remap, int z_lo, int z_hi, int first,
                          int count, int* out, int* grid)
{
  if (!plan || width < 1 || rows < 1 || ty < 1 || z_hi <= z_lo || first < 0 || count < 0 || (count && !out)) return 1;
  const int ntx = (width + kPair8Lanes - 1) / kPair8Lanes, nty = (rows + ty - 1) / ty;
  int v[9];
  for (int i = 0; i < 9; ++i) v[i] = static_cast<int>(plan[i]);
  const Pair8Cut cut = {v[0], v[1], v[2], v[3], v[4], v[5], v[6], v[7], v[8]};
  for (int i = 0; i < 9; i += 3)
    if (v[i] < 0 || (v[i] && (v[i + 1] < 1 || v[i + 2] < 1))) return 1;
  if (cut.tiles_a + cut.tiles_b + cut.tiles_c != pair8_tiles_per_chunk(ntx, nty, fold != 0)) return 1;
  if (grid) *grid = pair8_cut_grid(cut, xcd_remap);
  for (int i = 0; i < count; ++i) {
    Pair8Wg w;
    int* o = out + 6 * static_cast<size_t>(i);
    if (pair8_decode(first + i, cut, ntx, nty, fold != 0, xcd_remap, z_lo, z_hi, 0, w)) {
      o[0] = w.tile; o[1] = w.tx; o[2] = w.ty; o[3] = w.folded ? 1 : 0; o[4] = w.z0; o[5] = w.z1;
    } else {
      std::fill(o, o + 6, -1);
    }
  }
  return 0;
}

size_t f3d_max_warp_level(size_t width, size_t height, size_t depth, float scale_factor)
{
  return OpticalFlowBase::GetMaxWarpLevel(width, height, depth, scale_factor);
}

int f3d_level_geometry(size_t width, size_t height, size_t depth, float scale_factor, int level, f3d_size4* size,
                       float* hx, float* hy, float* hz)
{
  if (!size || !hx || !hy || !hz) return 1;
  DataSize4 original = {width, height, depth, 0};
  PyramidLevel lv = OpticalFlowBase::GetLevel(original, scale_factor, level);
  *size = {lv.size.width, lv.size.height, lv.size.depth, 0};
  *hx = lv.hx;
  *hy = lv.hy;
// ... 221 lines not shown
```

### cuda-flow3d_amd/host/operations.cpp

```cpp
#include "operations.h"

#include <algorithm>
#include <cmath>
#include <cstdio>
#include <utility>

#include "common_utils.h"
#include "hip_utils.h"
#include "solve_schedule.h"

extern "C" int f3d_solve_sweep_add(f3d_devptr frame_0, f3d_devptr frame_1, f3d_devptr flow_u, f3d_devptr flow_v, f3d_devptr flow_w,
                                   f3d_devptr flow_du, f3d_devptr flow_dv, f3d_devptr flow_dw, f3d_devptr phi, f3d_devptr ksi,
                                   size_t width, size_t height, size_t depth, float hx, float hy, float hz, float equation_alpha,
                                   f3d_devptr sum_u, f3d_devptr sum_v, f3d_devptr sum_w, const f3d_slab* slab) __attribute__((weak));


bool CudaOperationBase::IsInitialized() const
{
  if (!initialized_) std::printf("Error: Operation '%s' was not initialized.\n", name_);
  return initialized_;
}

void CudaOperationBase::Execute(OperationParameters&)
{
  std::printf("Warning: '%s' Execute() was not defined.\n", name_);
}

void CudaOperationBase::Destroy() { initialized_ = false; }

CudaOperationBase::~CudaOperationBase()
{
  if (initialized_) Destroy();
}

bool CudaOperationBase::InitializeContainer(const OperationParameters* params)
{
  initialized_ = false;
  if (!params) {
    std::printf("Operation: '%s'. Initialization parameters are missing.\n", GetName());
    return initialized_;
  }
  DataSize4 container_size;
  GET_PARAM_OR_RETURN_VALUE(*params, DataSize4, container_size, "container_size", initialized_);
  dev_container_size_ = container_size;
  f3d_size4 c = {container_size.width, container_size.height, container_size.depth, container_size.pitch};
  if (!CheckDeviceError(f3d_set_container(&c))) initialized_ = true;
  return initialized_;
}


void CudaOperationAdd::Execute(OperationParameters& params)
{
  if (!IsInitialized()) return;
  ProfilerRange range(GetName());
  DevicePtr operand_0, operand_1;
  DataSize4 data_size;
  GET_PARAM_OR_RETURN(params, DevicePtr, operand_0, "operand_0");
  GET_PARAM_OR_RETURN(params, DevicePtr, operand_1, "operand_1");
  GET_PARAM_OR_RETURN(params, DataSize4, data_size, "data_size");
  CheckDeviceError(f3d_add(operand_0, operand_1, data_size.width, data_size.height, data_size.depth, slab_));
}

namespace {
constexpr size_t kBatchMax = 3;
bool SameBox(const DataSize4& a, const DataSize4& b) { return a.width == b.width && a.height == b.height && a.depth == b.depth; }
}

void CudaOperationAdd::ExecuteBatch(OperationParameters* params, size_t count)
{
  if (!IsInitialized() || count == 0) return;
  DevicePtr a[kBatchMax], b[kBatchMax];
  DataSize4 size[kBatchMax];
  bool together = count <= kBatchMax;
  for (size_t i = 0; together && i < count; ++i) {
    void *p0 = params[i].GetValuePtr("operand_0"), *p1 = params[i].GetValuePtr("operand_1"), *ps = params[i].GetValuePtr("data_size");
    if (!p0 || !p1 || !ps) {
      together = false;
      break;
    }
    a[i] = *static_cast<DevicePtr*>(p0);
    b[i] = *static_cast<DevicePtr*>(p1);
    size[i] = *static_cast<DataSize4*>(ps);
    together = SameBox(size[i], size[0]);
    for (size_t j = 0; together && j < i; ++j) together = a[i] != a[j] && a[i] != b[j] && b[i] != a[j];
  }
  if (!together) {
    for (size_t i = 0; i < count; ++i) Execute(params[i]);
    return;
  }
  ProfilerRange range(GetName());
  CheckDeviceError(f3d_add_n(a, b, count, size[0].width, size[0].height, size[0].depth, slab_));
}


void CudaOperationStat::Execute(OperationParameters& params)
{
  if (!IsInitialized()) return;
// ... 311 lines not shown

void CudaOperationSolve::Destroy()
{
  FreeScratch();
  CudaOperationBase::Destroy();
}

void CudaOperationSolve::Execute(OperationParameters& params)
{
  if (!IsInitialized()) return;
  ProfilerRange range(GetName());

  DevicePtr dev_frame_0, dev_frame_1, dev_flow_u, dev_flow_v, dev_flow_w, dev_phi, dev_ksi;
  GET_PARAM_OR_RETURN(params, DevicePtr, dev_frame_0, "dev_frame_0");
  GET_PARAM_OR_RETURN(params, DevicePtr, dev_frame_1, "dev_frame_1");
  GET_PARAM_OR_RETURN(params, DevicePtr, dev_flow_u, "dev_flow_u");
  GET_PARAM_OR_RETURN(params, DevicePtr, dev_flow_v, "dev_flow_v");
  GET_PARAM_OR_RETURN(params, DevicePtr, dev_flow_w, "dev_flow_w");
  GET_PARAM_OR_RETURN(params, DevicePtr, dev_phi, "dev_phi");
  GET_PARAM_OR_RETURN(params, DevicePtr, dev_ksi, "dev_ksi");

  DevicePtr *du_ptr, *dv_ptr, *dw_ptr, *tdu_ptr, *tdv_ptr, *tdw_ptr;
  GET_PARAM_PTR_OR_RETURN(params, DevicePtr, du_ptr, "dev_flow_du");
  GET_PARAM_PTR_OR_RETURN(params, DevicePtr, dv_ptr, "dev_flow_dv");
  GET_PARAM_PTR_OR_RETURN(params, DevicePtr, dw_ptr, "dev_flow_dw");
  GET_PARAM_PTR_OR_RETURN(params, DevicePtr, tdu_ptr, "dev_temp_du");
  GET_PARAM_PTR_OR_RETURN(params, DevicePtr, tdv_ptr, "dev_temp_dv");
  GET_PARAM_PTR_OR_RETURN(params, DevicePtr, tdw_ptr, "dev_temp_dw");

  size_t outer_iterations_count, inner_iterations_count;
  float equation_alpha, equation_smoothness, equation_data, hx, hy, hz;
  DataSize4 data_size;
  GET_PARAM_OR_RETURN(params, size_t, outer_iterations_count, "outer_iterations_count");
  GET_PARAM_OR_RETURN(params, size_t, inner_iterations_count, "inner_iterations_count");
  GET_PARAM_OR_RETURN(params, float, equation_alpha, "equation_alpha");
  GET_PARAM_OR_RETURN(params, float, equation_smoothness, "equation_smoothness");
  GET_PARAM_OR_RETURN(params, float, equation_data, "equation_data");
  GET_PARAM_OR_RETURN(params, float, hx, "hx");
  GET_PARAM_OR_RETURN(params, float, hy, "hy");
  GET_PARAM_OR_RETURN(params, float, hz, "hz");
  GET_PARAM_OR_RETURN(params, DataSize4, data_size, "data_size");
  const bool fused = FusedSweepsEnabled() && SolveWeightsPlain(equation_alpha, hx, hy, hz);
  bool* flow_update = static_cast<bool*>(params.GetValuePtr("flow_update"));
  if (flow_update) *flow_update = false;

  {
    const DevicePtr increments[3] = {*du_ptr, *dv_ptr, *dw_ptr};
    f3d_slab all = {0, 0, 0};
    if (slab_) {
      const long top = static_cast<long>(slab_->z_base) + static_cast<long>(dev_container_size_.depth);
      all = {slab_->z_base, std::max(0, slab_->z_base), static_cast<int>(std::min<long>(static_cast<long>(data_size.depth), top))};
    }
    if (slab_ && all.z_lo >= all.z_hi) return;
    if (CheckDeviceError(f3d_clear_box_n(increments, 3, data_size.width, data_size.height, data_size.depth, slab_ ? &all : nullptr)))
      return;
  }

  f3d_event ev_start = nullptr, ev_stop = nullptr;
  if (!silent) {
    CheckDeviceError(f3d_event_create(&ev_start));
    CheckDeviceError(f3d_event_create(&ev_stop));
    CheckDeviceError(f3d_event_record(ev_start));
    Utils::PrintProgressBar(0.f);
    std::printf(" % 3.0f%%", 0.f);
  }

  const size_t w = data_size.width, h = data_size.height, d = data_size.depth;
  const int K = static_cast<int>(inner_iterations_count);
  const bool fuse_weights = fused && FusedPhiKsiEnabled() && outer_iterations_count > 1 && dev_container_size_.pitch % 256 == 0 &&
                            EnsureWeightScratch();
  const bool tri = fused && slab_ == nullptr && dev_container_size_.pitch % 256 == 0 && K >= 2 && ThreeStageLaunchesPay(w, h, d);
  const std::vector<SweepLaunch> cut_more = CutSweeps(K, fused, tri, fuse_weights), cut_last = CutSweeps(K, fused, tri, false);
  DevicePtr phi_cur = dev_phi, ksi_cur = dev_ksi, phi_nxt = phi_alt_, ksi_nxt = ksi_alt_;
  if (!cut_more.empty() && cut_more.back().next_weights && (outer_iterations_count - 1) % 2 == 1) {
    std::swap(phi_cur, phi_nxt);
    std::swap(ksi_cur, ksi_nxt);
  }
  bool weights_ready = false;
  const bool on_derivatives = !tri && fused && FrameDerivativesEnabled() && slab_ == nullptr && K >= 2 &&
                              f3d_fused_launches_march_along_y(w, h, d) == 0 &&
                              dev_container_size_.pitch % 256 == 0 && EnsureDerivativeScratch() &&
                              !CheckDeviceError(f3d_frame_derivatives(dev_frame_0, dev_frame_1, w, h, d, hx, hy, hz, fder_[0], fder_[1],
                                                                      fder_[2], fder_[3], nullptr));
  for (size_t i = 0; i < outer_iterations_count; ++i) {
    if (!weights_ready &&
        CheckDeviceError(f3d_phi_ksi(dev_frame_0, dev_frame_1, dev_flow_u, dev_flow_v, dev_flow_w, *du_ptr, *dv_ptr, *dw_ptr, w, h, d,
                                     hx, hy, hz, equation_smoothness, equation_data, phi_cur, ksi_cur, slab_)))
      return;
    weights_ready = false;
    const bool more = i + 1 < outer_iterations_count;
    for (const SweepLaunch& launch : more ? cut_more : cut_last) {
      const int group = launch.sweeps;
      const bool with_weights = launch.next_weights;
      int status;
      if (group == 3)
        status = f3d_solve_sweep3(dev_frame_0, dev_frame_1, dev_flow_u, dev_flow_v, dev_flow_w, *du_ptr, *dv_ptr, *dw_ptr, phi_cur, ksi_cur,
                                  w, h, d, hx, hy, hz, equation_alpha, *tdu_ptr, *tdv_ptr, *tdw_ptr, slab_);
      else if (group == 2 && with_weights)
        status = f3d_solve_sweep2_phi_ksi(dev_frame_0, dev_frame_1, dev_flow_u, dev_flow_v, dev_flow_w, *du_ptr, *dv_ptr, *dw_ptr, phi_cur,
                                          ksi_cur, w, h, d, hx, hy, hz, equation_alpha, equation_smoothness, equation_data, *tdu_ptr,
                                          *tdv_ptr, *tdw_ptr, phi_nxt, ksi_nxt, slab_);
      else if (group == 2 && on_derivatives)
        status = f3d_solve_sweep2_fd(fder_[0], fder_[1], fder_[2], fder_[3], dev_flow_u, dev_flow_v, dev_flow_w, *du_ptr, *dv_ptr,
                                     *dw_ptr, phi_cur, ksi_cur, w, h, d, hx, hy, hz, equation_alpha, *tdu_ptr, *tdv_ptr, *tdw_ptr, slab_);
      else if (group == 2)
        status = f3d_solve_sweep2(dev_frame_0, dev_frame_1, dev_flow_u, dev_flow_v, dev_flow_w, *du_ptr, *dv_ptr, *dw_ptr, phi_cur,
                                  ksi_cur, w, h, d, hx, hy, hz, equation_alpha, *tdu_ptr, *tdv_ptr, *tdw_ptr, slab_);
      else if (with_weights && on_derivatives)
        status = f3d_solve_sweep_phi_ksi_fd(fder_[0], fder_[1], fder_[2], fder_[3], dev_flow_u, dev_flow_v, dev_flow_w, *du_ptr,
                                            *dv_ptr, *dw_ptr, phi_cur, ksi_cur, w, h, d, hx, hy, hz, equation_alpha,
                                            equation_smoothness, equation_data, *tdu_ptr, *tdv_ptr, *tdw_ptr, phi_nxt, ksi_nxt, slab_);
      else if (with_weights)
        status = f3d_solve_sweep_phi_ksi(dev_frame_0, dev_frame_1, dev_flow_u, dev_flow_v, dev_flow_w, *du_ptr, *dv_ptr, *dw_ptr,
                                         phi_cur, ksi_cur, w, h, d, hx, hy, hz, equation_alpha, equation_smoothness, equation_data,
                                         *tdu_ptr, *tdv_ptr, *tdw_ptr, phi_nxt, ksi_nxt, slab_);
      else if (flow_update && f3d_solve_sweep_add && !more && launch.first + 1 == K) {
        status = f3d_solve_sweep_add(dev_frame_0, dev_frame_1, dev_flow_u, dev_flow_v, dev_flow_w, *du_ptr, *dv_ptr, *dw_ptr, phi_cur,
                                     ksi_cur, w, h, d, hx, hy, hz, equation_alpha, *tdu_ptr, *tdv_ptr, *tdw_ptr, slab_);
        *flow_update = status == 0;
      } else
        status = f3d_solve_sweep(dev_frame_0, dev_frame_1, dev_flow_u, dev_flow_v, dev_flow_w, *du_ptr, *dv_ptr, *dw_ptr, phi_cur,
                                 ksi_cur, w, h, d, hx, hy, hz, equation_alpha, *tdu_ptr, *tdv_ptr, *tdw_ptr, slab_);
      if (CheckDeviceError(status)) return;
      std::swap(*du_ptr, *tdu_ptr);
      std::swap(*dv_ptr, *tdv_ptr);
      std::swap(*dw_ptr, *tdw_ptr);
      if (with_weights) {
        std::swap(phi_cur, phi_nxt);
        std::swap(ksi_cur, ksi_nxt);
        weights_ready = true;
      }
    }
    if (!silent) {
      CheckDeviceError(f3d_stream_sync());
      const float complete = static_cast<float>(i + 1) / static_cast<float>(outer_iterations_count);
      Utils::PrintProgressBar(complete);
      std::printf(" % 3.0f%%", complete * 100);
    }
  }

  if (!silent) {
    float elapsed_ms = 0.f;
    CheckDeviceError(f3d_event_record(ev_stop));
    CheckDeviceError(f3d_event_sync(ev_stop));
    CheckDeviceError(f3d_event_elapsed_ms(&elapsed_ms, ev_start, ev_stop));
    Utils::PrintProgressBar(1.f);
    std::printf(" %8.4fs\n", elapsed_ms / 1000.);
    f3d_event_destroy(ev_start);
    f3d_event_destroy(ev_stop);
  }
}
```

### cuda-flow3d_amd/host/solve_schedule.cpp

```cpp
#include "solve_schedule.h"

#include <algorithm>
#include <cmath>

bool SolveWeightsPlain(float equation_alpha, float hx, float hy, float hz)
{
  for (float h : {hx, hy, hz}) {
    const float w = equation_alpha / (h * h);
    if (!(w - w == 0.f) || std::signbit(w)) return false;
  }
  return true;
}

std::vector<SweepLaunch> CutSweeps(int K, bool fused, bool tri, bool carry)
{
  std::vector<SweepLaunch> cut;
  for (int first = 0; first < K;) {
    const int left = K - first;
    int sweeps = fused ? std::min(left, tri ? 3 : 2) : 1;
    if (fused && tri && carry && left >= 2 && left <= 4) sweeps = left == 3 ? 1 : 2;
    cut.push_back({first, sweeps, false});
    first += sweeps;
  }
  if (fused && carry && !cut.empty()) cut.back().next_weights = cut.back().sweeps == 1 || (tri && cut.back().sweeps == 2);
  return cut;
}
```

### cuda-flow3d_amd/host/solve_schedule.h

```cpp
#ifndef F3D_HOST_SOLVE_SCHEDULE_H_
#define F3D_HOST_SOLVE_SCHEDULE_H_

#include <vector>

bool SolveWeightsPlain(float equation_alpha, float hx, float hy, float hz);

struct SweepLaunch {
  int first;
  int sweeps;
  bool next_weights;
};

std::vector<SweepLaunch> CutSweeps(int K, bool fused, bool tri, bool carry);

#endif
```

### include/f3d.h

```cpp
#ifndef F3D_H_
#define F3D_H_

#include <stddef.h>
#include <stdint.h>

#ifdef __cplusplus
extern "C" {
#endif

typedef uint64_t f3d_devptr;

typedef struct f3d_size4 {
  size_t width;
  size_t height;
  size_t depth;
  size_t pitch;
} f3d_size4;

typedef struct f3d_slab {
  int z_base;
  int z_lo;
  int z_hi;
} f3d_slab;

// ... 43 lines not shown
int f3d_host_register(void* ptr, size_t bytes);
int f3d_host_unregister(void* ptr);
int f3d_host_is_pinned(const void* ptr, int* yes);
int f3d_copy_d2d(f3d_devptr dst, f3d_devptr src, size_t bytes);
int f3d_set_container(const f3d_size4* container);
int f3d_get_container(f3d_size4* container);

int f3d_event_create(f3d_event* ev);
int f3d_event_record(f3d_event ev);
int f3d_event_sync(f3d_event ev);
int f3d_event_elapsed_ms(float* ms, f3d_event start, f3d_event stop);
int f3d_event_destroy(f3d_event ev);
int f3d_stream_sync(void);


int f3d_phi_ksi(f3d_devptr frame_0, f3d_devptr frame_1, f3d_devptr flow_u, f3d_devptr flow_v, f3d_devptr flow_w,
                f3d_devptr flow_du, f3d_devptr flow_dv, f3d_devptr flow_dw,
                size_t width, size_t height, size_t depth, float hx, float hy, float hz,
                float equation_smoothness, float equation_data, f3d_devptr phi, f3d_devptr ksi,
                const f3d_slab* slab);

int f3d_phi_ksi_zones(f3d_devptr frame_0, f3d_devptr frame_1, f3d_devptr flow_u, f3d_devptr flow_v, f3d_devptr flow_w,
                      f3d_devptr flow_du, f3d_devptr flow_dv, f3d_devptr flow_dw, size_t width, size_t height, size_t depth, float hx,
                      float hy, float hz, float equation_smoothness, float equation_data, f3d_devptr phi, f3d_devptr ksi,
                      const f3d_slab* zone_a, const f3d_slab* zone_b);

int f3d_solve_sweep(f3d_devptr frame_0, f3d_devptr frame_1, f3d_devptr flow_u, f3d_devptr flow_v, f3d_devptr flow_w,
                    f3d_devptr flow_du, f3d_devptr flow_dv, f3d_devptr flow_dw, f3d_devptr phi, f3d_devptr ksi,
                    size_t width, size_t height, size_t depth, float hx, float hy, float hz, float equation_alpha,
                    f3d_devptr temp_du, f3d_devptr temp_dv, f3d_devptr temp_dw, const f3d_slab* slab);

int f3d_solve_sweep_add(f3d_devptr frame_0, f3d_devptr frame_1, f3d_devptr flow_u, f3d_devptr flow_v, f3d_devptr flow_w,
                        f3d_devptr flow_du, f3d_devptr flow_dv, f3d_devptr flow_dw, f3d_devptr phi, f3d_devptr ksi,
                        size_t width, size_t height, size_t depth, float hx, float hy, float hz, float equation_alpha,
                        f3d_devptr sum_u, f3d_devptr sum_v, f3d_devptr sum_w, const f3d_slab* slab);

int f3d_solve_sweep2(f3d_devptr frame_0, f3d_devptr frame_1, f3d_devptr flow_u, f3d_devptr flow_v, f3d_devptr flow_w,
                     f3d_devptr flow_du, f3d_devptr flow_dv, f3d_devptr flow_dw, f3d_devptr phi, f3d_devptr ksi,
                     size_t width, size_t height, size_t depth, float hx, float hy, float hz, float equation_alpha,
                     f3d_devptr temp_du, f3d_devptr temp_dv, f3d_devptr temp_dw, const f3d_slab* slab);

int f3d_solve_sweep_phi_ksi(f3d_devptr frame_0, f3d_devptr frame_1, f3d_devptr flow_u, f3d_devptr flow_v, f3d_devptr flow_w,
                            f3d_devptr flow_du, f3d_devptr flow_dv, f3d_devptr flow_dw, f3d_devptr phi, f3d_devptr ksi,
                            size_t width, size_t height, size_t depth, float hx, float hy, float hz, float equation_alpha,
                            float equation_smoothness, float equation_data, f3d_devptr temp_du, f3d_devptr temp_dv,
                            f3d_devptr temp_dw, f3d_devptr phi_next, f3d_devptr ksi_next, const f3d_slab* slab);

int f3d_solve_sweep_phi_ksi_edges(f3d_devptr frame_0, f3d_devptr frame_1, f3d_devptr flow_u, f3d_devptr flow_v, f3d_devptr flow_w,
                                  f3d_devptr flow_du, f3d_devptr flow_dv, f3d_devptr flow_dw, f3d_devptr phi, f3d_devptr ksi,
                                  size_t width, size_t height, size_t depth, float hx, float hy, float hz, float equation_alpha,
                                  float equation_smoothness, float equation_data, f3d_devptr temp_du, f3d_devptr temp_dv,
                                  f3d_devptr temp_dw, f3d_devptr phi_next, f3d_devptr ksi_next, const f3d_slab* slab,
                                  int keep_below, int keep_above);

int f3d_fused_launches_march_along_y(size_t width, size_t height, size_t depth);

int f3d_solve_sweep3(f3d_devptr frame_0, f3d_devptr frame_1, f3d_devptr flow_u, f3d_devptr flow_v, f3d_devptr flow_w,
                     f3d_devptr flow_du, f3d_devptr flow_dv, f3d_devptr flow_dw, f3d_devptr phi, f3d_devptr ksi, size_t width,
                     size_t height, size_t depth, float hx, float hy, float hz, float equation_alpha, f3d_devptr temp_du,
                     f3d_devptr temp_dv, f3d_devptr temp_dw, const f3d_slab* slab);
int f3d_solve_sweep2_phi_ksi(f3d_devptr frame_0, f3d_devptr frame_1, f3d_devptr flow_u, f3d_devptr flow_v, f3d_devptr flow_w,
                             f3d_devptr flow_du, f3d_devptr flow_dv, f3d_devptr flow_dw, f3d_devptr phi, f3d_devptr ksi, size_t width,
                             size_t height, size_t depth, float hx, float hy, float hz, float equation_alpha,
                             float equation_smoothness, float equation_data, f3d_devptr temp_du, f3d_devptr temp_dv,
                             f3d_devptr temp_dw, f3d_devptr phi_next, f3d_devptr ksi_next, const f3d_slab* slab);

int f3d_frame_derivatives(f3d_devptr frame_0, f3d_devptr frame_1, size_t width, size_t height, size_t depth, float hx, float hy,
                          float hz, f3d_devptr fx, f3d_devptr fy, f3d_devptr fz, f3d_devptr ft, const f3d_slab* slab);
int f3d_solve_sweep2_fd(f3d_devptr fx, f3d_devptr fy, f3d_devptr fz, f3d_devptr ft, f3d_devptr flow_u, f3d_devptr flow_v, f3d_devptr flow_w,
                        f3d_devptr flow_du, f3d_devptr flow_dv, f3d_devptr flow_dw, f3d_devptr phi, f3d_devptr ksi, size_t width,
                        size_t height, size_t depth, float hx, float hy, float hz, float equation_alpha, f3d_devptr temp_du,
                        f3d_devptr temp_dv, f3d_devptr temp_dw, const f3d_slab* slab);
int f3d_solve_sweep_phi_ksi_fd(f3d_devptr fx, f3d_devptr fy, f3d_devptr fz, f3d_devptr ft, f3d_devptr flow_u, f3d_devptr flow_v,
                               f3d_devptr flow_w, f3d_devptr flow_du, f3d_devptr flow_dv, f3d_devptr flow_dw, f3d_devptr phi,
                               f3d_devptr ksi, size_t width, size_t height, size_t depth, float hx, float hy, float hz,
                               float equation_alpha, float equation_smoothness, float equation_data, f3d_devptr temp_du,
                               f3d_devptr temp_dv, f3d_devptr temp_dw, f3d_devptr phi_next, f3d_devptr ksi_next, const f3d_slab* slab);
int f3d_solve_sweep_phi_ksi_edges_fd(f3d_devptr fx, f3d_devptr fy, f3d_devptr fz, f3d_devptr ft, f3d_devptr flow_u, f3d_devptr flow_v,
                                     f3d_devptr flow_w, f3d_devptr flow_du, f3d_devptr flow_dv, f3d_devptr flow_dw, f3d_devptr phi,
                                     f3d_devptr ksi, size_t width, size_t height, size_t depth, float hx, float hy, float hz,
                                     float equation_alpha, float equation_smoothness, float equation_data, f3d_devptr temp_du,
                                     f3d_devptr temp_dv, f3d_devptr temp_dw, f3d_devptr phi_next, f3d_devptr ksi_next,
                                     const f3d_slab* slab, int keep_below, int keep_above);

int f3d_warp(f3d_devptr frame_0, f3d_devptr frame_1, f3d_devptr flow_u, f3d_devptr flow_v, f3d_devptr flow_w,
             size_t width, size_t height, size_t depth, float hx, float hy, float hz, f3d_devptr output,
             const f3d_slab* slab);

int f3d_resample_x(f3d_devptr input, f3d_devptr output, size_t out_width, size_t out_height, size_t out_depth,
                   size_t in_width, const f3d_slab* slab);
int f3d_resample_y(f3d_devptr input, f3d_devptr output, size_t out_width, size_t out_height, size_t out_depth,
                   size_t in_height, const f3d_slab* slab);
int f3d_resample_z(f3d_devptr input, f3d_devptr output, size_t out_width, size_t out_height, size_t out_depth,
                   size_t in_depth, const f3d_slab* slab_in, const f3d_slab* slab);

int f3d_add(f3d_devptr operand_0, f3d_devptr operand_1, size_t width, size_t height, size_t depth,
            const f3d_slab* slab);

int f3d_median(f3d_devptr input, size_t width, size_t height, size_t depth, size_t radius, f3d_devptr output,
               const f3d_slab* slab);

int f3d_resample_x_n(const f3d_devptr* inputs, const f3d_devptr* outputs, size_t count, size_t out_width, size_t out_height,
                     size_t out_depth, size_t in_width, const f3d_slab* slab);
int f3d_resample_y_n(const f3d_devptr* inputs, const f3d_devptr* outputs, size_t count, size_t out_width, size_t out_height,
                     size_t out_depth, size_t in_height, const f3d_slab* slab);
int f3d_resample_z_n(const f3d_devptr* inputs, const f3d_devptr* outputs, size_t count, size_t out_width, size_t out_height,
                     size_t out_depth, size_t in_depth, const f3d_slab* slab_in, const f3d_slab* slab);
int f3d_add_n(const f3d_devptr* operand_0, const f3d_devptr* operand_1, size_t count, size_t width, size_t height, size_t depth,
              const f3d_slab* slab);
int f3d_median_n(const f3d_devptr* inputs, size_t count, size_t width, size_t height, size_t depth, size_t radius,
                 const f3d_devptr* outputs, const f3d_slab* slab);
int f3d_clear_box_n(const f3d_devptr* volumes, size_t count, size_t width, size_t height, size_t depth, const f3d_slab* slab);

int f3d_set_conv_taps(const float* taps, size_t count);
int f3d_conv_rows(f3d_devptr dst, f3d_devptr src, size_t width, size_t height, size_t depth, size_t kernel_radius,
                  const f3d_slab* slab);
int f3d_conv_cols(f3d_devptr dst, f3d_devptr src, size_t width, size_t height, size_t depth, size_t kernel_radius,
                  const f3d_slab* slab);
int f3d_conv_slices(f3d_devptr dst, f3d_devptr src, size_t width, size_t height, size_t depth, size_t kernel_radius,
                    const f3d_slab* slab);
int f3d_conv_rows_cols(f3d_devptr dst, f3d_devptr src, size_t width, size_t height, size_t depth, size_t kernel_radius,
                       const f3d_slab* slab);

int f3d_selftest_weights(unsigned lo_bits, unsigned hi_bits, unsigned long long* checked, unsigned long long* excluded,
                         unsigned long long* mismatches, unsigned* first_mismatch);

int f3d_range_push(const char* name);
int f3d_range_pop(void);


enum { F3D_K_PHI_KSI = 0, F3D_K_SWEEP = 1, F3D_K_SWEEP2 = 2, F3D_K_SWEEP_PHI_KSI = 3, F3D_K_SWEEP3 = 4, F3D_K_SWEEP2_PHI_KSI = 5,
       F3D_K_COUNT = 6 };
int f3d_prof_enable(int enable);
int f3d_prof_reset(void);
int f3d_prof_select(unsigned kernel_mask);
int f3d_prof_read(int kernel, size_t min_voxels, double* total_ms, uint64_t* launches, double* total_voxels);


int f3d_comm_unique_id(void* id128);
int f3d_comm_init(const void* id128, int rank, int n_ranks);
int f3d_comm_destroy(void);
int f3d_comm_rank(int* rank, int* n_ranks);
int f3d_comm_info(int* backend, int* comm_ranks, int* comm_rank, int* comm_device, unsigned long long* sent_bytes,
                  unsigned long long* exchanges);
int f3d_pack_planes(f3d_devptr field, int plane0, int count, size_t width, size_t height, f3d_devptr staging,
                    size_t offset_floats);
int f3d_unpack_planes(f3d_devptr field, int plane0, int count, size_t width, size_t height, f3d_devptr staging,
                      size_t offset_floats);
int f3d_pack_segments(const f3d_devptr* fields, const int* plane0, const int* count, const size_t* offset_floats,
                      int n_segments, size_t width, size_t height, f3d_devptr staging);
int f3d_unpack_segments(const f3d_devptr* fields, const int* plane0, const int* count, const size_t* offset_floats,
                        int n_segments, size_t width, size_t height, f3d_devptr staging);
int f3d_copy_planes(f3d_devptr dst, int dst_plane0, f3d_devptr src, int src_plane0, int count, size_t width,
                    size_t height);
int f3d_copy_plane_segments(const f3d_devptr* dst, const int* dst_plane0, const f3d_devptr* src, const int* src_plane0, const int* count,
                            int n_segments, size_t width, size_t height);
int f3d_comm_sendrecv(f3d_devptr send_buf, const size_t* send_offset, const size_t* send_count, f3d_devptr recv_buf,
                      const size_t* recv_offset, const size_t* recv_count, const int* peers, int n_peers);
int f3d_comm_sendrecv_begin(f3d_devptr send_buf, const size_t* send_offset, const size_t* send_count, f3d_devptr recv_buf,
                            const size_t* recv_offset, const size_t* recv_count, const int* peers, int n_peers);
int f3d_comm_sendrecv_end(void);
int f3d_comm_timing(int enable);
int f3d_comm_mark(int what, int cls);
int f3d_comm_timing_read(int cls, double* total_us, unsigned long long* count, double* min_us, double* max_us,
                         unsigned long long* bytes);
int f3d_comm_allreduce_max_f32(float* value);
// ... 185 lines not shown
```

### include/f3d_host.h

```cpp
#ifndef F3D_HOST_H_
#define F3D_HOST_H_

#include "f3d.h"

#ifdef __cplusplus
extern "C" {
#endif

typedef struct f3d_flow_params {
  size_t warp_levels_count;
  float  warp_scale_factor;
  size_t outer_iterations_count;
  size_t inner_iterations_count;
  float  equation_alpha;
  float  equation_smoothness;
  float  equation_data;
  size_t median_radius;
  float  gaussian_sigma;
} f3d_flow_params;

typedef struct f3d_flow_s* f3d_flow;
typedef struct f3d_op_s* f3d_op;

void f3d_flow_default_params(f3d_flow_params* p);
// ... 39 lines not shown
int f3d_flow_polar_end(f3d_flow flow);

int f3d_flow_window_principal_compute(f3d_flow flow, int source, unsigned fields, unsigned radius, unsigned min_count,
                                      float* const out[10], f3d_principal_stats* stats);
int f3d_flow_window_principal_end(f3d_flow flow);
int f3d_flow_window_polar_compute(f3d_flow flow, int source, unsigned fields, unsigned radius, unsigned min_count, float* const out[7],
                                  f3d_polar_stats* stats);
int f3d_flow_window_polar_end(f3d_flow flow);

int f3d_flow_inverse_compute(f3d_flow flow, int source, unsigned iterations, float tolerance, float* const out[4],
                             f3d_inverse_stats* stats);
int f3d_flow_inverse_end(f3d_flow flow);

#define F3D_MATCH_WARPED 1u
#define F3D_MATCH_ZNCC 2u
#define F3D_MATCH_RMSD 4u
int f3d_flow_match_compute(f3d_flow flow, int source, unsigned fields, unsigned radius, float threshold, float* const out[3],
                           f3d_correlation_stats* stats);
int f3d_flow_match_end(f3d_flow flow);

int f3d_motion_solve(const struct f3d_motion_sums* sums, int model, f3d_motion_fit* fit);

int f3d_motion_solve_labels(const struct f3d_motion_sums* sums, size_t n_labels, int model, unsigned long long min_voxels,
                            const double volume_centre[3], f3d_motion_fit* fits, int* status);

int f3d_flow_motion_compute(f3d_flow flow, int source, int model, float min_zncc, float* const out[3], f3d_motion_fit* fit,
                            f3d_motion_residual* residual);
int f3d_flow_motion_end(f3d_flow flow);

int f3d_flow_label_motion_compute(f3d_flow flow, int source, const int* labels, size_t n_labels, int model, unsigned long long min_voxels,
                                  float* const out[3], f3d_motion_fit* fits, int* status, double* rms_after ,
                                  f3d_label_info* info );
int f3d_flow_label_motion_end(f3d_flow flow);

#define F3D_CONTACT_SMALL 1u
#define F3D_CONTACT_FLAT 2u
#define F3D_CONTACT_NOJUMP 4u
#define F3D_CONTACT_UNFITTED 8u
typedef struct f3d_contact_kin {
  double point[3], area, normal[3];
  double jump_normal, jump_slip, fit_normal, fit_slip;
  unsigned status;
} f3d_contact_kin;
int f3d_contact_kinematics(const struct f3d_contact* contacts, size_t n, const size_t dims[3], const f3d_motion_fit* fits ,
                           const int* status , size_t n_labels, unsigned long long min_faces, f3d_contact_kin* out);

int f3d_flow_contacts_compute(f3d_flow flow, int source, const int* labels , size_t n_labels,
                              const struct f3d_contact** contacts, size_t* count, f3d_contact_info* info);
int f3d_flow_contacts_end(f3d_flow flow);

int f3d_flow_labels_compute(f3d_flow flow, f3d_devptr frame , float lo, float hi, unsigned long long min_voxels,
                            const unsigned long long** sizes, size_t* count, f3d_component_info* info);
int f3d_flow_labels_split(f3d_flow flow, f3d_devptr frame , float lo, float hi, unsigned long long core_d2,
                          unsigned long long min_voxels, const unsigned long long** sizes, size_t* count, f3d_split_info* info);
int f3d_flow_labels_end(f3d_flow flow);
int f3d_flow_labels_download(f3d_flow flow, int* labels);

int f3d_flow_validate_compute(f3d_flow flow, int source, unsigned step, float eps, float threshold, unsigned min_neighbours,
                              unsigned mode, unsigned fill_passes, float min_zncc, float* const out[4], f3d_validate_stats* stats);
int f3d_flow_validate_end(f3d_flow flow);
const char* f3d_host_last_error(void);
int f3d_flow_destroy(f3d_flow flow);

int f3d_op_create(f3d_op* op, const char* name);
const char* f3d_op_name(f3d_op op);
int f3d_op_initialize(f3d_op op, const f3d_size4* container_size);
int f3d_op_execute(f3d_op op, const char* const* keys, void* const* value_ptrs, size_t count);
int f3d_op_execute_batch(f3d_op op, const char* const* keys, void* const* value_ptrs, const size_t* counts, size_t bags);
int f3d_op_set_slab(f3d_op op, const f3d_slab* slab);
int f3d_op_destroy(f3d_op op);

typedef struct f3d_volume_s* f3d_volume;
int f3d_volume_wrap(f3d_volume* vol, float* data, size_t width, size_t height, size_t depth);
void* f3d_volume_object(f3d_volume vol);
float* f3d_volume_data(f3d_volume vol);
int f3d_volume_destroy(f3d_volume vol);
int f3d_op_solve_p_last(f3d_op op, int* chunk, int* outer_per_pass, int* halo, size_t* passes, int* overlapped);
int f3d_op_solve_p_fused_weights(f3d_op op, int* fused);
int f3d_plan_solve_piecemeal(size_t budget_bytes, size_t width, size_t height, int depth, int inner_iterations, int outer_iterations,
                             int forced_outer_per_pass, int overlap_mode, int* chunk, int* outer_per_pass, int* halo, int* max_planes,
                             int* overlapped);
size_t f3d_piecemeal_budget_bytes(void);
int f3d_plan_sweeps(int inner, int fused, int tri, int carry, int* sweeps, int* next_weights, int capacity);
int f3d_pair8_plan(int width, int rows, int planes, int ty, int zc_limit, int per_round, int fold, long long* plan);
int f3d_pair8_decode(int width, int rows, int ty, int fold, const long long* plan, int xcd_remap, int z_lo, int z_hi, int first,
                     int count, int* out, int* grid);
int f3d_pair8_plan_wide(int width, int rows, int planes, int ty, int zc_limit, int per_round, int fold, long long* plan);
int f3d_pair8_decode_wide(int width, int rows, int ty, int fold, const long long* plan, int xcd_remap, int z_lo, int z_hi, int first,
                          int count, int* out, int* grid);

typedef struct f3d_pflow_s* f3d_pflow;
int f3d_pflow_create(f3d_pflow* flow);
int f3d_pflow_initialize(f3d_pflow flow, size_t width, size_t height, size_t depth);
int f3d_pflow_compute(f3d_pflow flow, const float* frame_0, const float* frame_1, size_t width, size_t height, size_t depth,
                      const f3d_flow_params* params, int silent, float* u, float* v, float* w, float* device_seconds);
int f3d_pflow_stats(f3d_pflow flow, size_t* solve_passes, size_t* streamed_levels, size_t* resident_levels);
int f3d_pflow_levels_registered_inside(f3d_pflow flow, size_t* levels);
int f3d_pflow_levels_with_constants_on_device(f3d_pflow flow, size_t* levels);
int f3d_pflow_originals_on_device(f3d_pflow flow, int* yes);
int f3d_pflow_set_full_pipeline(f3d_pflow flow, int enabled);
int f3d_pflow_set_resident(f3d_pflow flow, int enabled);
int f3d_pflow_operator_seconds(f3d_pflow flow, double* seconds6);
int f3d_pflow_destroy(f3d_pflow flow);

size_t f3d_max_warp_level(size_t width, size_t height, size_t depth, float scale_factor);
int f3d_level_geometry(size_t width, size_t height, size_t depth, float scale_factor, int level,
                       f3d_size4* size, float* hx, float* hy, float* hz);
int f3d_gaussian_taps(float sigma, float* taps, size_t capacity, size_t* radius);
int f3d_raw_read_u8(const char* path, size_t width, size_t height, size_t depth, float* out);
int f3d_raw_read_f32(const char* path, size_t width, size_t height, size_t depth, float* out);
int f3d_raw_write_u8(const char* path, const float* in, size_t width, size_t height, size_t depth);
int f3d_raw_write_f32(const char* path, const float* in, size_t width, size_t height, size_t depth);
int f3d_vtk_write_flow(const char* path, const float* u, const float* v, const float* w, size_t width, size_t height,
                       size_t depth);
int f3d_synth_pair(size_t width, size_t height, size_t depth, float* frame_0, float* frame_1);
int f3d_synth_planes(size_t width, size_t height, size_t depth, size_t z_lo, size_t z_hi, float* frame_0, float* frame_1,
                     float* frame_0_max);


typedef struct f3d_slabflow_s* f3d_slabflow;

int f3d_slabflow_create(f3d_slabflow* flow, int n_ranks, const int* local_ranks, int n_local, int halo_capacity);
int f3d_slabflow_initialize(f3d_slabflow flow, size_t width, size_t height, size_t depth);
int f3d_slabflow_compute(f3d_slabflow flow, const float* frame_0, const float* frame_1, const f3d_flow_params* params,
                         float* u, float* v, float* w);
int f3d_slabflow_upload(f3d_slabflow flow, const float* frame_0, const float* frame_1);
int f3d_slabflow_compute_resident(f3d_slabflow flow, const f3d_flow_params* params, float* device_seconds);
int f3d_slabflow_download(f3d_slabflow flow, float* u, float* v, float* w);
int f3d_slabflow_overlapped_iterations(f3d_slabflow flow, size_t* count);
int f3d_slabflow_batched_exchanges(f3d_slabflow flow, size_t* count);
int f3d_slabflow_gathered_warps(f3d_slabflow flow, size_t* count);
int f3d_slabflow_stage_exchanges(f3d_slabflow flow, size_t* count);
int f3d_slabflow_set_exchange_per_stage(f3d_slabflow flow, int per_stage);
int f3d_slabflow_destroy(f3d_slabflow flow);

int f3d_plan_owned(int depth, int rank, int n_ranks, int* lo, int* hi);
int f3d_plan_exchange(int depth, int rank, int n_ranks, int need_lo, int need_hi, int* peer, int* send_lo, int* send_hi,
                      int* recv_lo, int* recv_hi, int capacity);
int f3d_plan_resample_source(int in_depth, int out_depth, int out_lo, int out_hi, int* lo, int* hi);

#ifdef __cplusplus
}
#endif
#endif
```

Before: 74.84 Mvoxels/s.

## Add weights-first sweep schedule with fused phi/ksi+sweep and sweep2+add kernels

```diff
diff --git a/cuda-flow3d_amd/__init__.py b/cuda-flow3d_amd/__init__.py
--- a/cuda-flow3d_amd/__init__.py
+++ b/cuda-flow3d_amd/__init__.py
@@ -397,6 +397,7 @@
         "f3d_op_solve_p_fused_weights": [C.c_void_p, C.POINTER(C.c_int)],
         "f3d_plan_solve_piecemeal": [_sz, _sz, _sz, C.c_int, C.c_int, C.c_int, C.c_int, C.c_int] + [C.POINTER(C.c_int)] * 5,
         "f3d_plan_sweeps": [C.c_int] * 4 + [C.POINTER(C.c_int)] * 2 + [C.c_int],
+        "f3d_plan_sweeps_weights_first": [C.c_int] + [C.POINTER(C.c_int)] * 4 + [C.c_int],
         "f3d_pair8_plan": [C.c_int] * 7 + [C.POINTER(C.c_longlong)],
         "f3d_pair8_decode": [C.c_int] * 4 + [C.POINTER(C.c_longlong)] + [C.c_int] * 5 + [C.POINTER(C.c_int)] * 2,
         "f3d_pair8_plan_wide": [C.c_int] * 7 + [C.POINTER(C.c_longlong)],
@@ -477,6 +478,16 @@
                   "add the increments to the flow inside the last sweep")
 
 
+def solve_phi_ksi_sweep_fd_entry():
+    return _entry("f3d_solve_phi_ksi_sweep_fd", [_dp] * 10 + [_sz] * 3 + [C.c_float] * 6 + [_dp] * 5 + [_slabp],
+                  "compute the weights in front of a sweep")
+
+
+def solve_sweep2_add_fd_entry():
+    return _entry("f3d_solve_sweep2_add_fd", [_dp] * 12 + [_sz] * 3 + [C.c_float] * 4 + [_dp] * 3 + [_slabp],
+                  "add the increments to the flow inside the last two sweeps")
+
+
 def _compose_entry():
     return _entry("f3d_compose_flow", [_dp] * 6 + [_sz] * 3 + [C.POINTER(C.c_ulonglong)], "compose flows into a trajectory")
 
@@ -1464,6 +1475,15 @@
     return [(sweeps[i], bool(weights[i])) for i in range(n)]
 
 
+def plan_sweeps_weights_first(inner):
+    cap = max(1, inner)
+    start, sweeps, first, nxt = (C.c_int * cap)(), (C.c_int * cap)(), (C.c_int * cap)(), (C.c_int * cap)()
+    n = host().f3d_plan_sweeps_weights_first(inner, start, sweeps, first, nxt, cap)
+    if n < 0:
+        raise F3dError("f3d_plan_sweeps_weights_first failed")
+    return [(start[i], sweeps[i], bool(first[i]), bool(nxt[i])) for i in range(n)]
+
+
 Pair8Plan = collections.namedtuple("Pair8Plan", "A a b zc_a zc_b wgs cost tiles")
 
 
diff --git a/cuda-flow3d_amd/csrc/f3d_solve.hip b/cuda-flow3d_amd/csrc/f3d_solve.hip
--- a/cuda-flow3d_amd/csrc/f3d_solve.hip
+++ b/cuda-flow3d_amd/csrc/f3d_solve.hip
@@ -1510,6 +1510,74 @@
                   equation_data, out, slab, keep_below, keep_above);
 }
 
+namespace {
+int wpair8_fd(const char* who, bool weights_first, const f3d_devptr (&in)[12], size_t width, size_t height, size_t depth, float hx, float hy,
+              float hz, float alpha, float eps_s, float eps_d, const f3d_devptr (&out)[5], const f3d_slab* slab)
+{
+  if (slab) return f3d::fail("%s: whole levels only (no z-slab window)", who);
+  F3dGeo g;
+  if (!f3d::make_geo(&g, width, height, depth, nullptr, who)) return 1;
+  if (g.W < 2 || g.H < 2 || g.D < 2) return f3d::fail("%s: every dimension must be at least 2", who);
+  if (!pair_weights_finite(hx, hy, hz, alpha)) return f3d::fail("%s: alpha / h^2 must be finite and not negative (alpha %g, h %g %g %g)", who, alpha, hx, hy, hz);
+  if (g.pitch % 256 != 0) return f3d::fail("%s: the container pitch must be a multiple of 256 floats", who);
+  if (!pair8_enabled() || pair8_ymarch_rows(g) != 0) return f3d::fail("%s: the fused launches march along y on this level", who);
+  for (int i = 0; i < 5; ++i)
+    for (int k = 0; k < 12; ++k)
+      if (out[i] && out[i] == in[k]) return f3d::fail("%s: an output buffer is also an input (other tiles still read it)", who);
+  for (int i = 0; i < 5; ++i)
+    for (int k = i + 1; k < 5; ++k)
+      if (out[i] && out[i] == out[k]) return f3d::fail("%s: two outputs are the same buffer", who);
+  PairArgs a = {};
+  static const int plain_division = std::getenv("F3D_UDIV") && std::atoi(std::getenv("F3D_UDIV")) == 0;
+  a.plain_division = plain_division;
+  for (int i = 0; i < 12; ++i) a.in[i] = f3d_ptr<const float>(in[i]);
+  for (int i = 0; i < 5; ++i) a.out[i] = f3d_ptr<float>(out[i]);
+  a.hx = hx; a.hy = hy; a.hz = hz;
+  a.alpha = alpha;
+  a.eps_s = eps_s;
+  a.eps_d = eps_d;
+  const int kid = weights_first ? F3D_K_SWEEP_PHI_KSI : F3D_K_SWEEP2;
+  f3d::prof_begin(kid, static_cast<size_t>(g.W) * g.H * (g.z_hi - g.z_lo));
+  const int rows = pair8_rows(g);
+  if (weights_first) {
+    if (rows == 12) launch_pair8<PAIR_PS, 12, true>(a, g, tuning().zchunk, tuning().xcd_remap);
+    else if (rows == 4) launch_pair8<PAIR_PS, 4, true>(a, g, tuning().zchunk, tuning().xcd_remap);
+    else launch_pair8<PAIR_PS, 8, true>(a, g, tuning().zchunk, tuning().xcd_remap);
+  } else {
+    if (rows == 12) launch_pair8<PAIR_SSA, 12, true>(a, g, tuning().zchunk, tuning().xcd_remap);
+    else if (rows == 4) launch_pair8<PAIR_SSA, 4, true>(a, g, tuning().zchunk, tuning().xcd_remap);
+    else launch_pair8<PAIR_SSA, 8, true>(a, g, tuning().zchunk, tuning().xcd_remap);
+  }
+  f3d::prof_end(kid);
+  F3D_HIP(hipGetLastError());
+  return 0;
+}
+}
+
+int f3d_solve_phi_ksi_sweep_fd(f3d_devptr fx, f3d_devptr fy, f3d_devptr fz, f3d_devptr ft, f3d_devptr flow_u, f3d_devptr flow_v,
+                               f3d_devptr flow_w, f3d_devptr flow_du, f3d_devptr flow_dv, f3d_devptr flow_dw, size_t width, size_t height,
+                               size_t depth, float hx, float hy, float hz, float equation_alpha, float equation_smoothness,
+                               float equation_data, f3d_devptr phi_out, f3d_devptr ksi_out, f3d_devptr temp_du, f3d_devptr temp_dv,
+                               f3d_devptr temp_dw, const f3d_slab* slab)
+{
+  F3D_REQUIRE_READY("f3d_solve_phi_ksi_sweep_fd");
+  const f3d_devptr in[12] = {fx, fy, flow_u, flow_v, flow_w, flow_du, flow_dv, flow_dw, 0, 0, fz, ft};
+  const f3d_devptr out[5] = {temp_du, temp_dv, temp_dw, phi_out, ksi_out};
+  return wpair8_fd("f3d_solve_phi_ksi_sweep_fd", true, in, width, height, depth, hx, hy, hz, equation_alpha, equation_smoothness,
+                   equation_data, out, slab);
+}
+
+int f3d_solve_sweep2_add_fd(f3d_devptr fx, f3d_devptr fy, f3d_devptr fz, f3d_devptr ft, f3d_devptr flow_u, f3d_devptr flow_v,
+                            f3d_devptr flow_w, f3d_devptr flow_du, f3d_devptr flow_dv, f3d_devptr flow_dw, f3d_devptr phi, f3d_devptr ksi,
+                            size_t width, size_t height, size_t depth, float hx, float hy, float hz, float equation_alpha, f3d_devptr sum_u,
+                            f3d_devptr sum_v, f3d_devptr sum_w, const f3d_slab* slab)
+{
+  F3D_REQUIRE_READY("f3d_solve_sweep2_add_fd");
+  const f3d_devptr in[12] = {fx, fy, flow_u, flow_v, flow_w, flow_du, flow_dv, flow_dw, phi, ksi, fz, ft};
+  const f3d_devptr out[5] = {sum_u, sum_v, sum_w, 0, 0};
+  return wpair8_fd("f3d_solve_sweep2_add_fd", false, in, width, height, depth, hx, hy, hz, equation_alpha, 0.f, 0.f, out, slab);
+}
+
 int f3d_fused_launches_march_along_y(size_t width, size_t height, size_t depth)
 {
   F3dGeo g = {};
diff --git a/cuda-flow3d_amd/csrc/f3d_solve_pair8.h b/cuda-flow3d_amd/csrc/f3d_solve_pair8.h
--- a/cuda-flow3d_amd/csrc/f3d_solve_pair8.h
+++ b/cuda-flow3d_amd/csrc/f3d_solve_pair8.h
@@ -1,5 +1,5 @@
 
-enum { PAIR_SS = 0, PAIR_SP = 1 };
+enum { PAIR_SS = 0, PAIR_SP = 1, PAIR_PS = 2, PAIR_SSA = 3 };
 
 struct PairArgs {
   const float* in[12];
@@ -42,13 +42,13 @@
   if (a.plain_division) a.fdivs_ok = a.sdivs_ok = 0;
 }
 
-template <int TY, int NA = 10, bool FD = false, bool TIGHT = false>
+template <int TY, int NA = 10, bool FD = false, bool TIGHT = false, bool WF = false>
 struct Pair8Lds {
   static constexpr int NR = TY + (TIGHT ? 0 : 2);
   static constexpr int NJ = TY + (TIGHT ? 0 : 4);
   static constexpr int NK = (NJ + 3) / 4;
   static constexpr int NJP = NJ;
-  static constexpr int NS = FD ? 7 : NA;
+  static constexpr int NS = FD ? (WF ? 6 : 7) : NA;
   static constexpr int kHaloLanes = NS * 2 * NJ;
   static constexpr int NH = (kHaloLanes + 63) / 64;
   static constexpr int kRowFloats = NS * NJP * 64;
@@ -57,10 +57,10 @@
   static constexpr int kSlots = 3;
   static constexpr int kPerPlane = NS * NK + NH;
   static_assert(kPerPlane <= 63, "s_waitcnt vmcnt(kPerPlane): the counter has six bits");
-  static constexpr int NC = FD ? 5 : 0;
-  static constexpr int NRC = TY + 2;
+  static constexpr int NC = FD ? (WF ? 4 : 5) : 0;
+  static constexpr int NRC = WF ? TY : TY + 2;
   static constexpr int NKC = (NRC + 3) / 4;
-  static constexpr int kCHaloLanes = NC * 2 * TY;
+  static constexpr int kCHaloLanes = WF ? 0 : NC * 2 * TY;
   static constexpr int NHC = (kCHaloLanes + 63) / 64;
   static constexpr int kCRowFloats = NC * NRC * 64;
   static constexpr int kCHaloOff = kCRowFloats;
@@ -169,6 +169,50 @@
   }
 }
 
+__device__ __forceinline__ void weights_first_stage1(float (&q)[9], bool with_ksi, float fx, float fy, float fz, float ft, float du,
+                                                     float dv_c, float dw, const SolveDivs& dv, float eps_s2, float eps_d2, float& phi,
+                                                     float& ksi, bool counts, bool fast_weights)
+{
+  if (__builtin_expect(dv.ok && udiv_all_safe(q), 1)) {
+#pragma unroll
+    for (int c = 0; c < 3; ++c) {
+      q[3 * c + 0] = udiv(q[3 * c + 0], dv.x2);
+      q[3 * c + 1] = udiv(q[3 * c + 1], dv.y2);
+      q[3 * c + 2] = udiv(q[3 * c + 2], dv.z2);
+    }
+  } else {
+#pragma unroll
+    for (int c = 0; c < 3; ++c) {
+      q[3 * c + 0] = q[3 * c + 0] / dv.x2.d;
+      q[3 * c + 1] = q[3 * c + 1] / dv.y2.d;
+      q[3 * c + 2] = q[3 * c + 2] / dv.z2.d;
+    }
+  }
+  const float dux = q[0], duy = q[1], duz = q[2], dvx = q[3], dvy = q[4], dvz = q[5], dwx = q[6], dwy = q[7], dwz = q[8];
+  const float a_phi = dux * dux + duy * duy + duz * duz + dvx * dvx + dvy * dvy + dvz * dvz + dwx * dwx + dwy * dwy + dwz * dwz + eps_s2;
+  float s_phi, s_ksi = 1.f, a_ksi = 1.f, w_ksi = 0.f;
+  const float w_phi = weight_fast(a_phi, s_phi);
+  bool lane_ok = weight_fast_ok(a_phi, s_phi);
+  if (with_ksi) {
+    const float J11 = fx * fx, J22 = fy * fy, J33 = fz * fz;
+    const float J12 = fx * fy, J13 = fx * fz, J23 = fy * fz;
+    const float J14 = fx * ft, J24 = fy * ft, J34 = fz * ft, J44 = ft * ft;
+    float s = (J11 * du + J12 * dv_c + J13 * dw + J14) * du + (J12 * du + J22 * dv_c + J23 * dw + J24) * dv_c +
+              (J13 * du + J23 * dv_c + J33 * dw + J34) * dw + (J14 * du + J24 * dv_c + J34 * dw + J44);
+    s = static_cast<float>(s > 0) * s;
+    a_ksi = s + eps_d2;
+    w_ksi = weight_fast(a_ksi, s_ksi);
+    lane_ok = lane_ok && weight_fast_ok(a_ksi, s_ksi);
+  }
+  if (__builtin_expect(fast_weights && __builtin_amdgcn_ballot_w64(counts && !lane_ok) == 0, 1)) {
+    phi = w_phi;
+    ksi = w_ksi;
+  } else {
+    phi = weight_ieee(a_phi);
+    ksi = with_ksi ? weight_ieee(a_ksi) : 0.f;
+  }
+}
+
 
 template <int MODE, int TY, int ABL, bool FD, bool YM, bool TIGHT, bool FOLDS = false>
 __device__ __forceinline__ void pair8_body(const PairArgs& a, const F3dGeo& g, const Pair8Cut& cut, int ntx, int nty, int xcd_remap)
@@ -176,19 +220,23 @@
   static_assert(!FOLDS || (!YM && !TIGHT && ABL == 0), "two row bands per tile: z-marching product builds only");
   static_assert(!(YM && FD), "the frame-derivative launchers march along z only");
   static_assert(!TIGHT || (YM && ABL == 0), "a tile without halo rows holds every row of the volume: thin volumes marched along y");
+  constexpr bool PS = MODE == PAIR_PS;
+  constexpr bool SSM = MODE == PAIR_SS || MODE == PAIR_SSA;
+  static_assert((!PS && MODE != PAIR_SSA) || (FD && !YM && !TIGHT && ABL == 0), "k_wpair8: frame-derivative z-marching product builds only");
   constexpr int RH = TIGHT ? 0 : 1;
   const int RDIM = YM ? g.D : g.H;
   const int MDIM = YM ? g.H : g.D;
   const int m_lo = YM ? 0 : g.z_lo, m_hi = YM ? g.H : g.z_hi;
   constexpr int NA = FD ? 12 : 10;
-  using L = Pair8Lds<TY, NA, FD, TIGHT>;
+  using L = Pair8Lds<TY, NA, FD, TIGHT, PS>;
   constexpr int NR = L::NR, NJ = L::NJ, NK = L::NK, NJP = L::NJP, NH = L::NH;
   static_assert(TY <= 32, "the column wave holds one halo voxel per lane: 2 x TY <= 64");
   __shared__ __attribute__((aligned(16))) float ring[L::kSlots][L::kSlotFloats];
   __shared__ __attribute__((aligned(16))) float cring[L::kCSlots][L::kCSlotFloats];
   constexpr int SB = FD ? 2 : 0;
-  __shared__ float img1[2][3][NR][kLanes];
-  __shared__ float hc1[2][3][2][32];
+  constexpr int NI = PS ? 4 : 3;
+  __shared__ float img1[2][NI][NR][kLanes];
+  __shared__ float hc1[2][NI][2][32];
   __shared__ float img3[(ABL & 64) ? 3 : 1][(ABL & 64) ? NR : 1][(ABL & 64) ? kLanes : 1];
 
   Pair8Wg wg;
@@ -227,7 +275,7 @@
     __builtin_amdgcn_s_setprio(3);
     const float* base[NA];
 #pragma unroll
-    for (int i = 0; i < NA; ++i) base[i] = uniform_ptr(a.in[i] + base_off);
+    for (int i = 0; i < NA; ++i) base[i] = (PS && (i == 8 || i == 9)) ? nullptr : uniform_ptr(a.in[i] + base_off);
     const bool bandb = FOLD && (lane & 15) >= 8;
     const int seg = bandb ? (lane & 15) - 8 : (lane & 15);
     unsigned rowb[NK];
@@ -275,8 +323,9 @@
       for (int h = 0; h < NH; ++h)
         if (hv[h]) dma16_lane(hptr[h] + (poff >> 2), slot + L::kHaloOff + h * 256);
     };
-    constexpr int NKC = FD ? L::NKC : 1, NHC = FD ? L::NHC : 1;
-    constexpr int kCIn[5] = {0, 1, 9, 10, 11};
+    constexpr int NKC = FD ? L::NKC : 1, NHC = FD && L::NHC > 0 ? L::NHC : 1;
+    constexpr int kCIn[5] = {0, 1, PS ? 10 : 9, PS ? 11 : 10, 11};
+    constexpr int CR0 = PS ? 0 : 1;
     unsigned crowb[NKC];
     bool crowv[NKC];
     const float* chptr[NHC];
@@ -286,7 +335,7 @@
       for (int k = 0; k < NKC; ++k) {
         const int j = 4 * k + (lane >> 4);
         crowv[k] = j < L::NRC;
-        const int yrow = f3d_clampi(f3d_mir(y0 + (bandb ? TY : 0) - 1 + (crowv[k] ? j : 0), RDIM), 0, RDIM - 1);
+        const int yrow = f3d_clampi(f3d_mir(y0 + (bandb ? TY : 0) - CR0 + (crowv[k] ? j : 0), RDIM), 0, RDIM - 1);
         crowb[k] = static_cast<unsigned>(yrow) * row_b + static_cast<unsigned>(x0 + 4 * seg) * 4u;
       }
 #pragma unroll
@@ -299,7 +348,7 @@
         const int j = lq % TY;
         const float* b = base[kCIn[0]];
 #pragma unroll
-        for (int i = 1; i < 5; ++i)
+        for (int i = 1; i < (FD ? L::NC : 1); ++i)
           if (arr == i) b = base[kCIn[i]];
         const int yrow = f3d_clampi(f3d_mir(y0 + (FOLD && s ? TY : 0) + j, RDIM), 0, RDIM - 1);
         const int xc = FOLD ? x0 - 4 : s == 0 ? (left_face ? 0 : x0 - 4) : (right_face ? x0 + kLanes - 4 : x0 + kLanes);
@@ -312,7 +361,7 @@
         const int zz = f3d_mir(p, MDIM);
         const unsigned poff = static_cast<unsigned>(__builtin_amdgcn_readfirstlane(static_cast<int>(static_cast<unsigned>(zz - zb) * plane_b)));
 #pragma unroll
-        for (int i = 0; i < 5; ++i) {
+        for (int i = 0; i < L::NC; ++i) {
 #pragma unroll
           for (int k = 0; k < NKC; ++k)
             if (L::NRC % 4 == 0 || crowv[k]) dma16(base[kCIn[i]], crowb[k] + poff, slot + (i * L::NRC + 4 * k) * kLanes);
@@ -353,7 +402,7 @@
   fdivs.x4 = UDiv{a.r4[0], a.d4[0]}; fdivs.y4 = UDiv{a.r4[1], a.d4[1]}; fdivs.z4 = UDiv{a.r4[2], a.d4[2]};
   fdivs.ok = a.fdivs_ok != 0;
   SolveDivs sdivs = {};
-  if (MODE == PAIR_SP) {
+  if (MODE == PAIR_SP || PS) {
     sdivs.x2 = UDiv{a.r2[0], a.d2[0]}; sdivs.y2 = UDiv{a.r2[1], a.d2[1]}; sdivs.z2 = UDiv{a.r2[2], a.d2[2]};
     sdivs.x4 = fdivs.x4; sdivs.y4 = fdivs.y4; sdivs.z4 = fdivs.z4;
     sdivs.ok = a.sdivs_ok != 0;
@@ -390,7 +439,7 @@
 
   float* obase[5];
 #pragma unroll
-  for (int i = 0; i < 5; ++i) obase[i] = (i < 3 || MODE == PAIR_SP) ? uniform_ptr(a.out[i] + base_off) : nullptr;
+  for (int i = 0; i < 5; ++i) obase[i] = (i < 3 || MODE == PAIR_SP || PS) ? uniform_ptr(a.out[i] + base_off) : nullptr;
   auto rowoff = [&](int yrow, int zz) __attribute__((always_inline)) {
     return static_cast<unsigned>(__builtin_amdgcn_readfirstlane(
         static_cast<int>(static_cast<unsigned>(zz - zb) * plane_b + static_cast<unsigned>(yrow) * row_b)));
@@ -587,7 +636,7 @@
         pN.D[6] = rxp.w - rxm.w; pN.D[7] = dY.w; pN.D[8] = dZ.w;
       }
     }
-    const S3 sN = MODE == PAIR_SS ? S3{C.u + r_du, C.v + r_dv, C.w + r_dw} : S3{r_du, r_dv, r_dw};
+    const S3 sN = SSM ? S3{C.u + r_du, C.v + r_dv, C.w + r_dw} : S3{r_du, r_dv, r_dw};
     if (do1 && !(ABL & 8)) {
       if constexpr (CW) {
         if (cactive) {
@@ -639,9 +688,15 @@
         o0 = xm.u + xp.v + ym.w + kC.J12;
         o1 = yp.u + zm.v + zp.w + kC.d1;
         o2 = xm.w + yp.v + zp.u + kC.pw[0] + hC_dv + hC_dw;
-      } else if (MODE == PAIR_SS)
+      } else if (SSM)
+      {
         sweep_stage2(kC, xm, xp, YM ? zm : ym, YM ? zp : yp, YM ? ym : zm, YM ? yp : zp, hC_dv, hC_dw, o0, o1, o2);
-      else
+        if constexpr (MODE == PAIR_SSA) {
+          o0 = kC.U + o0;
+          o1 = kC.V + o1;
+          o2 = kC.W + o2;
+        }
+      } else
         phi_ksi_stage2(pC, xm, xp, YM ? zm : ym, YM ? zp : yp, YM ? ym : zm, YM ? yp : zp, hC.u, hC.v, hC.w, sdivs, a.eps_s2,
                        a.eps_d2, o0, o1, owner, a.plain_division == 0);
     }
@@ -670,7 +725,7 @@
     pC = pN;
     if (do2 && owner) {
       const unsigned off = xb + rowoff(yy, t);
-      if (MODE == PAIR_SS) {
+      if (SSM) {
         gst(obase[0], off, o0);
         gst(obase[1], off, o1);
         gst(obase[2], off, o2);
@@ -680,6 +735,164 @@
       }
     }
     fetch_neighbours(colw_c, Sp);
+  };
+
+
+  auto row_raw_ps = [&](PlaneRegs& p, const float* slot, int j, bool centre, const float* cs) __attribute__((always_inline)) {
+    const float* d = slot + j * kLanes + lane;
+    constexpr int st = NJP * kLanes;
+    p.u = d[0 * st]; p.v = d[1 * st]; p.w = d[2 * st];
+    p.su = d[3 * st]; p.dv = d[4 * st]; p.dw = d[5 * st];
+    p.ksi = p.su;
+    if (centre) {
+      const float* c = cs + (j - 2) * kLanes + lane;
+      constexpr int ct = L::NRC * kLanes;
+      p.f0 = c[0 * ct]; p.f1 = c[1 * ct]; p.fz = c[2 * ct]; p.ft = c[3 * ct];
+    }
+  };
+  auto halo_raw_ps = [&](PlaneRegs& p, const float* slot, int s, int j, int e) __attribute__((always_inline)) {
+    const float* d = slot + L::kHaloOff + (s * NJ + j) * 4 + e;
+    constexpr int st = 2 * NJ * 4;
+    p.u = d[0 * st]; p.v = d[1 * st]; p.w = d[2 * st];
+    p.su = d[3 * st]; p.dv = d[4 * st]; p.dw = d[5 * st];
+    p.ksi = p.su;
+  };
+  S3 nXd = {0.f, 0.f, 0.f}, nInd = {0.f, 0.f, 0.f};
+  float phM = 0.f, phC = 0.f, ksC = 0.f;
+  auto fetch_ps = [&](auto colw_c, const float* S) __attribute__((always_inline)) {
+    constexpr bool CW = decltype(colw_c)::value;
+    PlaneRegs T0, T1, T2;
+    if constexpr (CW) {
+      PlaneRegs T;
+      const float* d = S + jc * kLanes + (side ? (FOLD ? 32 : kLanes - 1) : 0);
+      constexpr int st = NJP * kLanes;
+      T.u = d[0 * st]; T.v = d[1 * st]; T.w = d[2 * st]; T.su = d[3 * st]; T.dv = d[4 * st]; T.dw = d[5 * st];
+      nInr = {T.u, T.v, T.w};
+      nInd = {T.su, T.dv, T.dw};
+      halo_raw_ps(T0, S, side, jc_m, e_near);
+      halo_raw_ps(T1, S, side, jc_p, e_near);
+      halo_raw_ps(T2, S, side, jc, e_far);
+    } else {
+      row_raw_ps(T0, S, jr_m, false, nullptr);
+      row_raw_ps(T1, S, jr_p, false, nullptr);
+      halo_raw_ps(T2, S, side, jr, e_near);
+    }
+    nDy = {((T1.u - T0.u) + T1.su) - T0.su, ((T1.v - T0.v) + T1.dv) - T0.dv, ((T1.w - T0.w) + T1.dw) - T0.dw};
+    nXr = {T2.u, T2.v, T2.w};
+    nXd = {T2.su, T2.dv, T2.dw};
+  };
+  auto step_ps = [&](auto colw_c, auto slot_c, PlaneRegs& M, PlaneRegs& C, PlaneRegs& P, int q) __attribute__((always_inline)) {
+    constexpr bool CW = decltype(colw_c)::value;
+    constexpr int SLOT = decltype(slot_c)::value;
+    if constexpr (TY > 8) lane = fresh_lane();
+    const int band = FOLD ? lane >> 5 : 0;
+    __syncthreads();
+    const float* Sp = &ring[SLOT][0];
+    const float* Cp = &cring[(q + 1 - qs) & 1][0];
+    const bool do1 = q <= qe;
+    const int b = q & 1;
+    if constexpr (CW) halo_raw_ps(P, Sp, side, jc, e_near);
+    else row_raw_ps(P, Sp, jr, core, Cp);
+    plane_finish(P);
+
+    S3 rxm, rxp, dxm, dxp;
+    int vx, vy;
+    if constexpr (CW) {
+      rxm = !FOLD && side ? nInr : nXr;
+      rxp = !FOLD && side ? nXr : nInr;
+      dxm = !FOLD && side ? nInd : nXd;
+      dxp = !FOLD && side ? nXd : nInd;
+      vx = cx;
+      vy = cy;
+      if (cx == g.W - 1) {
+        rxp = rxm;
+        dxp = dxm;
+      }
+    } else {
+      rxm = {left_or(C.u, nXr.u), left_or(C.v, nXr.v), left_or(C.w, nXr.w)};
+      rxp = {lane_right_or(C.u, nXr.u), lane_right_or(C.v, nXr.v), lane_right_or(C.w, nXr.w)};
+      dxm = {left_or(C.ksi, nXd.u), left_or(C.dv, nXd.v), left_or(C.dw, nXd.w)};
+      dxp = {lane_right_or(C.ksi, nXd.u), lane_right_or(C.dv, nXd.v), lane_right_or(C.dw, nXd.w)};
+      vx = x;
+      vy = band ? y + TY : y;
+      if (tile_at_x_face) {
+        if (x == 0) {
+          rxm = rxp;
+          dxm = dxp;
+        }
+        if (x == g.W - 1) {
+          rxp = rxm;
+          dxp = dxm;
+        }
+      }
+    }
+    float nq[9] = {((rxp.u - rxm.u) + dxp.u) - dxm.u, nDy.u, ((P.u - M.u) + P.ksi) - M.ksi,
+                   ((rxp.v - rxm.v) + dxp.v) - dxm.v, nDy.v, ((P.v - M.v) + P.dv) - M.dv,
+                   ((rxp.w - rxm.w) + dxp.w) - dxm.w, nDy.w, ((P.w - M.w) + P.dw) - M.dw};
+    const bool counts = do1 && vx >= 0 && vx < g.W && vy >= 0 && vy < RDIM && (!CW || cactive);
+    float phi_q = 0.f, ksi_q = 0.f;
+    weights_first_stage1(nq, !CW && core, C.f0, C.f1, C.fz, C.ft, C.ksi, C.dv, C.dw, sdivs, a.eps_s2, a.eps_d2, phi_q, ksi_q, counts,
+                         a.plain_division == 0);
+    if (do1) {
+      if constexpr (CW) {
+        if (cactive) {
+          hc1[b][0][side][crow] = C.su;
+          hc1[b][1][side][crow] = C.sv;
+          hc1[b][2][side][crow] = C.sw;
+          hc1[b][3][side][crow] = phi_q;
+        }
+      } else {
+        img1[b][0][r][lane] = C.su;
+        img1[b][1][r][lane] = C.sv;
+        img1[b][2][r][lane] = C.sw;
+        img1[b][3][r][lane] = phi_q;
+      }
+    }
+    if (!CW && do1 && owner && q >= z0 && q < z1) {
+      const unsigned off = xb + rowoff(yy, q);
+      gst(obase[3], off, phi_q);
+      gst(obase[4], off, ksi_q);
+    }
+
+    const int t = q - 1;
+    const bool do2 = !CW && core && t >= z0;
+    float o0 = 0.f, o1 = 0.f, o2 = 0.f;
+    if (do2) {
+      const int pb = t & 1;
+      const int im = band ? r_ymb : r_ym, ip = band ? r_ypb : r_yp;
+      Face6 ym = {}, yp = {}, xm = {}, xp = {}, zm = {}, zp = {}, cf = {};
+      ym.v[LSU] = img1[pb][0][im][lane]; ym.v[LSV] = img1[pb][1][im][lane]; ym.v[LSW] = img1[pb][2][im][lane]; ym.v[LPHI] = img1[pb][3][im][lane];
+      yp.v[LSU] = img1[pb][0][ip][lane]; yp.v[LSV] = img1[pb][1][ip][lane]; yp.v[LSW] = img1[pb][2][ip][lane]; yp.v[LPHI] = img1[pb][3][ip][lane];
+      const float eu = hc1[pb][0][side][r - RH], ev = hc1[pb][1][side][r - RH], ew = hc1[pb][2][side][r - RH], ep = hc1[pb][3][side][r - RH];
+      cf.v[LSU] = M.su; cf.v[LSV] = M.sv; cf.v[LSW] = M.sw; cf.v[LPHI] = phC;
+      xm.v[LSU] = left_or(M.su, eu); xm.v[LSV] = left_or(M.sv, ev); xm.v[LSW] = left_or(M.sw, ew); xm.v[LPHI] = left_or(phC, ep);
+      xp.v[LSU] = lane_right_or(M.su, eu); xp.v[LSV] = lane_right_or(M.sv, ev); xp.v[LSW] = lane_right_or(M.sw, ew);
+      xp.v[LPHI] = lane_right_or(phC, ep);
+      zm.v[LSU] = hM.u; zm.v[LSV] = hM.v; zm.v[LSW] = hM.w; zm.v[LPHI] = phM;
+      zp.v[LSU] = C.su; zp.v[LSV] = C.sv; zp.v[LSW] = C.sw; zp.v[LPHI] = phi_q;
+      if (tile_at_x_face) {
+        if (x == 0) xm = xp;
+        if (x == g.W - 1) xp = xm;
+      }
+      if (t == 0) zm = zp;
+      if (t == MDIM - 1) zp = zm;
+      Carry kU;
+      sweep_stage1<true, true>(xm, xp, ym, yp, zm, zp, cf.v, M.u, M.v, M.w, M.dv, M.dw, ksC, a.hx, a.hy, a.hz, fdivs, a.alpha, vx < g.W - 1,
+                               vx > 0, vy < RDIM - 1, vy > 0, t < MDIM - 1, t > 0, o0, o1, o2, kU, M.f0, M.f1, M.fz, M.ft, tile_at_x_face,
+                               a.w[0], a.w[1], a.w[2]);
+    }
+    asm volatile("" ::"v"(o0), "v"(o1), "v"(o2), "v"(phi_q));
+    hM = {M.su, M.sv, M.sw};
+    phM = phC;
+    phC = phi_q;
+    ksC = ksi_q;
+    if (do2 && owner) {
+      const unsigned off = xb + rowoff(yy, t);
+      gst(obase[0], off, o0);
+      gst(obase[1], off, o1);
+      gst(obase[2], off, o2);
+    }
+    fetch_ps(colw_c, Sp);
   };
 
   __syncthreads();
@@ -691,7 +904,15 @@
   using Slot2 = std::integral_constant<int, 2>;
   auto march = [&](auto colw_c) __attribute__((always_inline)) {
     constexpr bool CW = decltype(colw_c)::value;
-    if constexpr (CW) {
+    if constexpr (PS) {
+      if constexpr (CW) {
+        halo_raw_ps(A, Sm, side, jc, e_near);
+        halo_raw_ps(B, S0, side, jc, e_near);
+      } else {
+        row_raw_ps(A, Sm, jr, false, nullptr);
+        row_raw_ps(B, S0, jr, core, &cring[0][0]);
+      }
+    } else if constexpr (CW) {
       halo_raw(A, Sm, side, jc, e_near, false);
       halo_raw(B, S0, side, jc, e_near, true, &cring[0][0]);
     } else {
@@ -700,15 +921,26 @@
     }
     plane_finish(A);
     plane_finish(B);
-    fetch_neighbours(colw_c, S0);
     int q = qs;
-    for (; q + 2 <= q_end; q += 3) {
-      step(colw_c, Slot2{}, A, B, Cc, q);
-      step(colw_c, Slot0{}, B, Cc, A, q + 1);
-      step(colw_c, Slot1{}, Cc, A, B, q + 2);
-    }
-    if (q <= q_end) step(colw_c, Slot2{}, A, B, Cc, q);
-    if (q + 1 <= q_end) step(colw_c, Slot0{}, B, Cc, A, q + 1);
+    if constexpr (PS) {
+      fetch_ps(colw_c, S0);
+      for (; q + 2 <= q_end; q += 3) {
+        step_ps(colw_c, Slot2{}, A, B, Cc, q);
+        step_ps(colw_c, Slot0{}, B, Cc, A, q + 1);
+        step_ps(colw_c, Slot1{}, Cc, A, B, q + 2);
+      }
+      if (q <= q_end) step_ps(colw_c, Slot2{}, A, B, Cc, q);
+      if (q + 1 <= q_end) step_ps(colw_c, Slot0{}, B, Cc, A, q + 1);
+    } else {
+      fetch_neighbours(colw_c, S0);
+      for (; q + 2 <= q_end; q += 3) {
+        step(colw_c, Slot2{}, A, B, Cc, q);
+        step(colw_c, Slot0{}, B, Cc, A, q + 1);
+        step(colw_c, Slot1{}, Cc, A, B, q + 2);
+      }
+      if (q <= q_end) step(colw_c, Slot2{}, A, B, Cc, q);
+      if (q + 1 <= q_end) step(colw_c, Slot0{}, B, Cc, A, q + 1);
+    }
   };
   if (colw) march(std::true_type{});
   else march(std::false_type{});
@@ -724,6 +956,11 @@
 __global__ __launch_bounds__(kLanes*(TY + 4)) void k_pair8(PairArgs a, F3dGeo g, Pair8Cut cut, int ntx, int nty, int xcd_remap)
 {
   pair8_body<MODE, TY, ABL, FD, YM, false, FOLDS>(a, g, cut, ntx, nty, xcd_remap);
+}
+template <int MODE, int TY, bool FOLDS>
+__global__ __launch_bounds__(kLanes*(TY + 4)) void k_wpair8(PairArgs a, F3dGeo g, Pair8Cut cut, int ntx, int nty, int xcd_remap)
+{
+  pair8_body<MODE, TY, 0, true, false, false, FOLDS>(a, g, cut, ntx, nty, xcd_remap);
 }
 template <int MODE, int TY>
 __global__ __launch_bounds__(kLanes*(TY + 2)) __attribute__((amdgpu_waves_per_eu(4))) void k_pair8t(PairArgs a, F3dGeo g, Pair8Cut cut, int ntx,
@@ -800,30 +1037,36 @@
   if (force_zchunk > 0) cut = pair8_uniform_cut(tiles, planes, std::min(force_zchunk, zc_limit));
   const dim3 grid(pair8_cut_grid(cut, xcd_remap), 1, 1), block(kLanes, TY + (TIGHT ? 2 : 4), 1);
   auto go = [&](auto kern) { hipLaunchKernelGGL(kern, grid, block, 0, f3d::stream(), a, g, cut, ntx, nty, xcd_remap); };
-  if constexpr (!YM) {
-    if (fold) return go(k_pair8<MODE, TY, 0, FD, false, true>);
-  }
-  if constexpr (YM && TIGHT) return go(k_pair8t<MODE, TY>);
-  else if constexpr (YM) return go(k_pair8<MODE, TY, 0, false, true>);
-  else if constexpr (FD) return go(k_pair8<MODE, TY, 0, true>);
-  else {
+  if constexpr (MODE == PAIR_PS || MODE == PAIR_SSA) {
+    static_assert(FD && !YM && !TIGHT, "k_wpair8");
+    if (fold) return go(k_wpair8<MODE, TY, true>);
+    return go(k_wpair8<MODE, TY, false>);
+  } else {
+    if constexpr (!YM) {
+      if (fold) return go(k_pair8<MODE, TY, 0, FD, false, true>);
+    }
+    if constexpr (YM && TIGHT) return go(k_pair8t<MODE, TY>);
+    else if constexpr (YM) return go(k_pair8<MODE, TY, 0, false, true>);
+    else if constexpr (FD) return go(k_pair8<MODE, TY, 0, true>);
+    else {
 #ifdef F3D_LAB
-    if constexpr (TY == 12) {
-      if (abl == 16) return go(k_pair8<MODE, TY, 16>);
-    }
-    if constexpr (MODE == PAIR_SS) {
-      if (abl == 1) return go(k_pair8<MODE, TY, 1>);
-      if (abl == 2) return go(k_pair8<MODE, TY, 2>);
-      if (abl == 3) return go(k_pair8<MODE, TY, 3>);
-      if (abl == 4) return go(k_pair8<MODE, TY, 4>);
-      if (abl == 8) return go(k_pair8<MODE, TY, 8>);
-      if (abl == 40) return go(k_pair8<MODE, TY, 40>);
-      if constexpr (TY <= 8) {
-        if (abl == 64) return go(k_pair8<MODE, TY, 64>);
-      }
-    }
+      if constexpr (TY == 12) {
+        if (abl == 16) return go(k_pair8<MODE, TY, 16>);
+      }
+      if constexpr (MODE == PAIR_SS) {
+        if (abl == 1) return go(k_pair8<MODE, TY, 1>);
+        if (abl == 2) return go(k_pair8<MODE, TY, 2>);
+        if (abl == 3) return go(k_pair8<MODE, TY, 3>);
+        if (abl == 4) return go(k_pair8<MODE, TY, 4>);
+        if (abl == 8) return go(k_pair8<MODE, TY, 8>);
+        if (abl == 40) return go(k_pair8<MODE, TY, 40>);
+        if constexpr (TY <= 8) {
+          if (abl == 64) return go(k_pair8<MODE, TY, 64>);
+        }
+      }
 #endif
-    go(k_pair8<MODE, TY, 0>);
+      go(k_pair8<MODE, TY, 0>);
+    }
   }
 }
 
diff --git a/cuda-flow3d_amd/host/hip_utils.cpp b/cuda-flow3d_amd/host/hip_utils.cpp
--- a/cuda-flow3d_amd/host/hip_utils.cpp
+++ b/cuda-flow3d_amd/host/hip_utils.cpp
@@ -47,6 +47,12 @@
   return on;
 }
 
+bool WeightsFirstEnabled()
+{
+  const char* e = std::getenv("F3D_WEIGHTS_FIRST");
+  return !(e && e[0] == '0');
+}
+
 bool FrameDerivativesEnabled()
 {
   static const bool on = [] {
diff --git a/cuda-flow3d_amd/host/hip_utils.h b/cuda-flow3d_amd/host/hip_utils.h
--- a/cuda-flow3d_amd/host/hip_utils.h
+++ b/cuda-flow3d_amd/host/hip_utils.h
@@ -30,6 +30,7 @@
 bool FusedSweepsEnabled();
 bool FusedPhiKsiEnabled();
 bool FrameDerivativesEnabled();
+bool WeightsFirstEnabled();
 bool ThreeStageLaunchesPay(size_t width, size_t height, size_t depth);
 
 #endif
diff --git a/cuda-flow3d_amd/host/host_capi.cpp b/cuda-flow3d_amd/host/host_capi.cpp
--- a/cuda-flow3d_amd/host/host_capi.cpp
+++ b/cuda-flow3d_amd/host/host_capi.cpp
@@ -764,6 +764,19 @@
   return static_cast<int>(cut.size());
 }
 
+int f3d_plan_sweeps_weights_first(int inner, int* first, int* sweeps, int* weights_first, int* next_weights, int capacity)
+{
+  const std::vector<SweepLaunch> cut = CutSweepsWeightsFirst(inner);
+  if (static_cast<int>(cut.size()) > capacity || (!cut.empty() && (!first || !sweeps || !weights_first || !next_weights))) return -1;
+  for (size_t i = 0; i < cut.size(); ++i) {
+    first[i] = cut[i].first;
+    sweeps[i] = cut[i].sweeps;
+    weights_first[i] = cut[i].weights_first ? 1 : 0;
+    next_weights[i] = cut[i].next_weights ? 1 : 0;
+  }
+  return static_cast<int>(cut.size());
+}
+
 int f3d_pair8_plan(int width, int rows, int planes, int ty, int zc_limit, int per_round, int fold, long long* plan)
 {
   if (!plan || width < 1 || rows < 1 || planes < 1 || ty < 1 || zc_limit < 1) return 1;
diff --git a/cuda-flow3d_amd/host/operations.cpp b/cuda-flow3d_amd/host/operations.cpp
--- a/cuda-flow3d_amd/host/operations.cpp
+++ b/cuda-flow3d_amd/host/operations.cpp
@@ -13,6 +13,18 @@
                                    f3d_devptr flow_du, f3d_devptr flow_dv, f3d_devptr flow_dw, f3d_devptr phi, f3d_devptr ksi,
                                    size_t width, size_t height, size_t depth, float hx, float hy, float hz, float equation_alpha,
                                    f3d_devptr sum_u, f3d_devptr sum_v, f3d_devptr sum_w, const f3d_slab* slab) __attribute__((weak));
+
+extern "C" int f3d_solve_phi_ksi_sweep_fd(f3d_devptr fx, f3d_devptr fy, f3d_devptr fz, f3d_devptr ft, f3d_devptr flow_u, f3d_devptr flow_v,
+                                          f3d_devptr flow_w, f3d_devptr flow_du, f3d_devptr flow_dv, f3d_devptr flow_dw, size_t width,
+                                          size_t height, size_t depth, float hx, float hy, float hz, float equation_alpha,
+                                          float equation_smoothness, float equation_data, f3d_devptr phi_out, f3d_devptr ksi_out,
+                                          f3d_devptr temp_du, f3d_devptr temp_dv, f3d_devptr temp_dw, const f3d_slab* slab)
+    __attribute__((weak));
+extern "C" int f3d_solve_sweep2_add_fd(f3d_devptr fx, f3d_devptr fy, f3d_devptr fz, f3d_devptr ft, f3d_devptr flow_u, f3d_devptr flow_v,
+                                       f3d_devptr flow_w, f3d_devptr flow_du, f3d_devptr flow_dv, f3d_devptr flow_dw, f3d_devptr phi,
+                                       f3d_devptr ksi, size_t width, size_t height, size_t depth, float hx, float hy, float hz,
+                                       float equation_alpha, f3d_devptr sum_u, f3d_devptr sum_v, f3d_devptr sum_w, const f3d_slab* slab)
+    __attribute__((weak));
 
 
 bool CudaOperationBase::IsInitialized() const
@@ -490,46 +502,64 @@
                               dev_container_size_.pitch % 256 == 0 && EnsureDerivativeScratch() &&
                               !CheckDeviceError(f3d_frame_derivatives(dev_frame_0, dev_frame_1, w, h, d, hx, hy, hz, fder_[0], fder_[1],
                                                                       fder_[2], fder_[3], nullptr));
-  for (size_t i = 0; i < outer_iterations_count; ++i) {
-    if (!weights_ready &&
+  bool weights_first = on_derivatives && WeightsFirstEnabled() && f3d_solve_phi_ksi_sweep_fd && f3d_solve_sweep2_add_fd;
+  const std::vector<SweepLaunch> cut_first = CutSweepsWeightsFirst(K);
+  enum { kDone, kFailed, kDeclined };
+  auto iteration = [&](size_t i, bool first) -> int {
+    const bool more = i + 1 < outer_iterations_count;
+    const DevicePtr phi_use = first ? dev_phi : phi_cur, ksi_use = first ? dev_ksi : ksi_cur;
+    if (!first && !weights_ready &&
         CheckDeviceError(f3d_phi_ksi(dev_frame_0, dev_frame_1, dev_flow_u, dev_flow_v, dev_flow_w, *du_ptr, *dv_ptr, *dw_ptr, w, h, d,
-                                     hx, hy, hz, equation_smoothness, equation_data, phi_cur, ksi_cur, slab_)))
-      return;
+                                     hx, hy, hz, equation_smoothness, equation_data, phi_use, ksi_use, slab_)))
+      return kFailed;
     weights_ready = false;
-    const bool more = i + 1 < outer_iterations_count;
-    for (const SweepLaunch& launch : more ? cut_more : cut_last) {
+    for (const SweepLaunch& launch : first ? cut_first : more ? cut_more : cut_last) {
       const int group = launch.sweeps;
       const bool with_weights = launch.next_weights;
+      const bool last_launch = !more && launch.first + launch.sweeps == K;
       int status;
-      if (group == 3)
-        status = f3d_solve_sweep3(dev_frame_0, dev_frame_1, dev_flow_u, dev_flow_v, dev_flow_w, *du_ptr, *dv_ptr, *dw_ptr, phi_cur, ksi_cur,
+      if (launch.weights_first) {
+        status = f3d_solve_phi_ksi_sweep_fd(fder_[0], fder_[1], fder_[2], fder_[3], dev_flow_u, dev_flow_v, dev_flow_w, *du_ptr, *dv_ptr,
+                                            *dw_ptr, w, h, d, hx, hy, hz, equation_alpha, equation_smoothness, equation_data, phi_use,
+                                            ksi_use, *tdu_ptr, *tdv_ptr, *tdw_ptr, slab_);
+        if (status != 0 && i == 0) return kDeclined;
+      } else if (group == 3)
+        status = f3d_solve_sweep3(dev_frame_0, dev_frame_1, dev_flow_u, dev_flow_v, dev_flow_w, *du_ptr, *dv_ptr, *dw_ptr, phi_use, ksi_use,
                                   w, h, d, hx, hy, hz, equation_alpha, *tdu_ptr, *tdv_ptr, *tdw_ptr, slab_);
       else if (group == 2 && with_weights)
-        status = f3d_solve_sweep2_phi_ksi(dev_frame_0, dev_frame_1, dev_flow_u, dev_flow_v, dev_flow_w, *du_ptr, *dv_ptr, *dw_ptr, phi_cur,
-                                          ksi_cur, w, h, d, hx, hy, hz, equation_alpha, equation_smoothness, equation_data, *tdu_ptr,
+        status = f3d_solve_sweep2_phi_ksi(dev_frame_0, dev_frame_1, dev_flow_u, dev_flow_v, dev_flow_w, *du_ptr, *dv_ptr, *dw_ptr, phi_use,
+                                          ksi_use, w, h, d, hx, hy, hz, equation_alpha, equation_smoothness, equation_data, *tdu_ptr,
                                           *tdv_ptr, *tdw_ptr, phi_nxt, ksi_nxt, slab_);
-      else if (group == 2 && on_derivatives)
-        status = f3d_solve_sweep2_fd(fder_[0], fder_[1], fder_[2], fder_[3], dev_flow_u, dev_flow_v, dev_flow_w, *du_ptr, *dv_ptr,
-                                     *dw_ptr, phi_cur, ksi_cur, w, h, d, hx, hy, hz, equation_alpha, *tdu_ptr, *tdv_ptr, *tdw_ptr, slab_);
-      else if (group == 2)
-        status = f3d_solve_sweep2(dev_frame_0, dev_frame_1, dev_flow_u, dev_flow_v, dev_flow_w, *du_ptr, *dv_ptr, *dw_ptr, phi_cur,
-                                  ksi_cur, w, h, d, hx, hy, hz, equation_alpha, *tdu_ptr, *tdv_ptr, *tdw_ptr, slab_);
+      else if (group == 2 && on_derivatives) {
+        status = 1;
+        if (first && flow_update && last_launch) {
+          status = f3d_solve_sweep2_add_fd(fder_[0], fder_[1], fder_[2], fder_[3], dev_flow_u, dev_flow_v, dev_flow_w, *du_ptr, *dv_ptr,
+                                           *dw_ptr, phi_use, ksi_use, w, h, d, hx, hy, hz, equation_alpha, *tdu_ptr, *tdv_ptr, *tdw_ptr,
+                                           slab_);
+          *flow_update = status == 0;
+        }
+        if (status != 0)
+          status = f3d_solve_sweep2_fd(fder_[0], fder_[1], fder_[2], fder_[3], dev_flow_u, dev_flow_v, dev_flow_w, *du_ptr, *dv_ptr,
+                                       *dw_ptr, phi_use, ksi_use, w, h, d, hx, hy, hz, equation_alpha, *tdu_ptr, *tdv_ptr, *tdw_ptr, slab_);
+      } else if (group == 2)
+        status = f3d_solve_sweep2(dev_frame_0, dev_frame_1, dev_flow_u, dev_flow_v, dev_flow_w, *du_ptr, *dv_ptr, *dw_ptr, phi_use,
+                                  ksi_use, w, h, d, hx, hy, hz, equation_alpha, *tdu_ptr, *tdv_ptr, *tdw_ptr, slab_);
       else if (with_weights && on_derivatives)
         status = f3d_solve_sweep_phi_ksi_fd(fder_[0], fder_[1], fder_[2], fder_[3], dev_flow_u, dev_flow_v, dev_flow_w, *du_ptr,
-                                            *dv_ptr, *dw_ptr, phi_cur, ksi_cur, w, h, d, hx, hy, hz, equation_alpha,
+                                            *dv_ptr, *dw_ptr, phi_use, ksi_use, w, h, d, hx, hy, hz, equation_alpha,
                                             equation_smoothness, equation_data, *tdu_ptr, *tdv_ptr, *tdw_ptr, phi_nxt, ksi_nxt, slab_);
       else if (with_weights)
         status = f3d_solve_sweep_phi_ksi(dev_frame_0, dev_frame_1, dev_flow_u, dev_flow_v, dev_flow_w, *du_ptr, *dv_ptr, *dw_ptr,
-                                         phi_cur, ksi_cur, w, h, d, hx, hy, hz, equation_alpha, equation_smoothness, equation_data,
+                                         phi_use, ksi_use, w, h, d, hx, hy, hz, equation_alpha, equation_smoothness, equation_data,
                                          *tdu_ptr, *tdv_ptr, *tdw_ptr, phi_nxt, ksi_nxt, slab_);
-      else if (flow_update && f3d_solve_sweep_add && !more && launch.first + 1 == K) {
-        status = f3d_solve_sweep_add(dev_frame_0, dev_frame_1, dev_flow_u, dev_flow_v, dev_flow_w, *du_ptr, *dv_ptr, *dw_ptr, phi_cur,
-                                     ksi_cur, w, h, d, hx, hy, hz, equation_alpha, *tdu_ptr, *tdv_ptr, *tdw_ptr, slab_);
+      else if (flow_update && f3d_solve_sweep_add && last_launch) {
+        status = f3d_solve_sweep_add(dev_frame_0, dev_frame_1, dev_flow_u, dev_flow_v, dev_flow_w, *du_ptr, *dv_ptr, *dw_ptr, phi_use,
+                                     ksi_use, w, h, d, hx, hy, hz, equation_alpha, *tdu_ptr, *tdv_ptr, *tdw_ptr, slab_);
         *flow_update = status == 0;
       } else
-        status = f3d_solve_sweep(dev_frame_0, dev_frame_1, dev_flow_u, dev_flow_v, dev_flow_w, *du_ptr, *dv_ptr, *dw_ptr, phi_cur,
-                                 ksi_cur, w, h, d, hx, hy, hz, equation_alpha, *tdu_ptr, *tdv_ptr, *tdw_ptr, slab_);
-      if (CheckDeviceError(status)) return;
+        status = f3d_solve_sweep(dev_frame_0, dev_frame_1, dev_flow_u, dev_flow_v, dev_flow_w, *du_ptr, *dv_ptr, *dw_ptr, phi_use,
+                                 ksi_use, w, h, d, hx, hy, hz, equation_alpha, *tdu_ptr, *tdv_ptr, *tdw_ptr, slab_);
+      if (CheckDeviceError(status)) return kFailed;
       std::swap(*du_ptr, *tdu_ptr);
       std::swap(*dv_ptr, *tdv_ptr);
       std::swap(*dw_ptr, *tdw_ptr);
@@ -539,6 +569,15 @@
         weights_ready = true;
       }
     }
+    return kDone;
+  };
+  for (size_t i = 0; i < outer_iterations_count; ++i) {
+    int outcome = iteration(i, weights_first);
+    if (outcome == kDeclined) {
+      weights_first = false;
+      outcome = iteration(i, false);
+    }
+    if (outcome != kDone) return;
     if (!silent) {
       CheckDeviceError(f3d_stream_sync());
       const float complete = static_cast<float>(i + 1) / static_cast<float>(outer_iterations_count);
diff --git a/cuda-flow3d_amd/host/solve_schedule.cpp b/cuda-flow3d_amd/host/solve_schedule.cpp
--- a/cuda-flow3d_amd/host/solve_schedule.cpp
+++ b/cuda-flow3d_amd/host/solve_schedule.cpp
@@ -25,3 +25,16 @@
   if (fused && carry && !cut.empty()) cut.back().next_weights = cut.back().sweeps == 1 || (tri && cut.back().sweeps == 2);
   return cut;
 }
+
+std::vector<SweepLaunch> CutSweepsWeightsFirst(int K)
+{
+  std::vector<SweepLaunch> cut;
+  if (K < 1) return cut;
+  cut.push_back({0, 1, false, true});
+  for (int first = 1; first < K;) {
+    const int sweeps = std::min(K - first, 2);
+    cut.push_back({first, sweeps, false, false});
+    first += sweeps;
+  }
+  return cut;
+}
diff --git a/cuda-flow3d_amd/host/solve_schedule.h b/cuda-flow3d_amd/host/solve_schedule.h
--- a/cuda-flow3d_amd/host/solve_schedule.h
+++ b/cuda-flow3d_amd/host/solve_schedule.h
@@ -9,8 +9,11 @@
   int first;
   int sweeps;
   bool next_weights;
+  bool weights_first = false;
 };
 
 std::vector<SweepLaunch> CutSweeps(int K, bool fused, bool tri, bool carry);
 
+std::vector<SweepLaunch> CutSweepsWeightsFirst(int K);
+
 #endif
diff --git a/include/f3d.h b/include/f3d.h
--- a/include/f3d.h
+++ b/include/f3d.h
@@ -149,6 +149,16 @@
                                      float equation_alpha, float equation_smoothness, float equation_data, f3d_devptr temp_du,
                                      f3d_devptr temp_dv, f3d_devptr temp_dw, f3d_devptr phi_next, f3d_devptr ksi_next,
                                      const f3d_slab* slab, int keep_below, int keep_above);
+
+int f3d_solve_phi_ksi_sweep_fd(f3d_devptr fx, f3d_devptr fy, f3d_devptr fz, f3d_devptr ft, f3d_devptr flow_u, f3d_devptr flow_v,
+                               f3d_devptr flow_w, f3d_devptr flow_du, f3d_devptr flow_dv, f3d_devptr flow_dw, size_t width, size_t height,
+                               size_t depth, float hx, float hy, float hz, float equation_alpha, float equation_smoothness,
+                               float equation_data, f3d_devptr phi_out, f3d_devptr ksi_out, f3d_devptr temp_du, f3d_devptr temp_dv,
+                               f3d_devptr temp_dw, const f3d_slab* slab);
+int f3d_solve_sweep2_add_fd(f3d_devptr fx, f3d_devptr fy, f3d_devptr fz, f3d_devptr ft, f3d_devptr flow_u, f3d_devptr flow_v,
+                            f3d_devptr flow_w, f3d_devptr flow_du, f3d_devptr flow_dv, f3d_devptr flow_dw, f3d_devptr phi, f3d_devptr ksi,
+                            size_t width, size_t height, size_t depth, float hx, float hy, float hz, float equation_alpha, f3d_devptr sum_u,
+                            f3d_devptr sum_v, f3d_devptr sum_w, const f3d_slab* slab);
 
 int f3d_warp(f3d_devptr frame_0, f3d_devptr frame_1, f3d_devptr flow_u, f3d_devptr flow_v, f3d_devptr flow_w,
              size_t width, size_t height, size_t depth, float hx, float hy, float hz, f3d_devptr output,
diff --git a/include/f3d_host.h b/include/f3d_host.h
--- a/include/f3d_host.h
+++ b/include/f3d_host.h
@@ -145,6 +145,7 @@
                              int* overlapped);
 size_t f3d_piecemeal_budget_bytes(void);
 int f3d_plan_sweeps(int inner, int fused, int tri, int carry, int* sweeps, int* next_weights, int capacity);
+int f3d_plan_sweeps_weights_first(int inner, int* first, int* sweeps, int* weights_first, int* next_weights, int capacity);
 int f3d_pair8_plan(int width, int rows, int planes, int ty, int zc_limit, int per_round, int fold, long long* plan);
 int f3d_pair8_decode(int width, int rows, int ty, int fold, const long long* plan, int xcd_remap, int z_lo, int z_hi, int first,
                      int count, int* out, int* grid);
```

After: 76.58 Mvoxels/s (median of 6 runs). 2.3% higher.
